# snap-stanford/pretrain-gnns

Hardware: NVIDIA H100
Metric: graphs/sec 5-layer GIN-300 fwd+bwd on ZINC-shaped batches (higher is better)
Workload: dtype tf32x3

## Files before the change

### include/pgnn_b200.h

```cpp
#ifndef PGNN_B200_H
#define PGNN_B200_H

#include <stdint.h>

#ifdef __cplusplus
extern "C" {
#endif

#define PGNN_API __attribute__((visibility("default")))

#define PGNN_OK 0
#define PGNN_EINVAL (-1)
#define PGNN_ECUDA (-2)
#define PGNN_EWORKSPACE (-3)
#define PGNN_EUNSUPPORTED (-4)

#define PGNN_DEVERR_NODE_ID 1u
#define PGNN_DEVERR_ATOM_CODE 2u
#define PGNN_DEVERR_BOND_CODE 4u
#define PGNN_DEVERR_LABEL 8u
#define PGNN_DEVERR_GATHER 16u

#define PGNN_AGG_SUM 0
#define PGNN_AGG_MEAN 1
#define PGNN_AGG_GCN 2

PGNN_API int pgnn_version(void);
PGNN_API const char* pgnn_error_string(int code);
PGNN_API int pgnn_last_cuda_error(void);
PGNN_API int pgnn_device_error_flags(int clear);
PGNN_API int pgnn_device_sm_count(int device);
PGNN_API int64_t pgnn_kernel_launch_count(void);
PGNN_API int pgnn_profile_enable(int on);
PGNN_API int64_t pgnn_profile_read(char* buf, int64_t buflen);


PGNN_API int64_t pgnn_bucket_workspace_bytes(int64_t num_keys, int64_t num_buckets);
PGNN_API int pgnn_bucket(const int64_t* keys, int64_t key_stride, int64_t num_keys, int64_t num_buckets,
                         const int64_t* vals, int64_t val_stride,
                         int32_t* rowptr, int32_t* order, int32_t* vals_out,
                         void* workspace, int64_t workspace_bytes, void* stream);

PGNN_API int64_t pgnn_graph_prep_workspace_bytes(int64_t num_nodes, int64_t num_edges);
PGNN_API int pgnn_graph_prep(const int64_t* edge_index, int64_t num_edges, int64_t num_nodes,
                             int32_t* rowptr_t, int32_t* nbr_t, int32_t* eid_t,
                             int32_t* rowptr_s, int32_t* nbr_s, int32_t* eid_s,
                             void* workspace, int64_t workspace_bytes, void* stream);

PGNN_API int pgnn_gcn_dinv(const int32_t* rowptr_t, int64_t num_nodes, float* dinv, void* stream);

PGNN_API int pgnn_chem_edge_summary(const int64_t* edge_attr , const int32_t* rowptr_t,
                                    const int32_t* nbr_t, const int32_t* eid_t, int64_t num_nodes,
                                    int mode, const float* dinv, float* S , void* stream);
PGNN_API int pgnn_bio_edge_summary(const float* edge_attr , const int32_t* rowptr_t,
                                   const int32_t* nbr_t, const int32_t* eid_t, int64_t num_nodes,
                                   int mode, const float* dinv, float* S , void* stream);

PGNN_API int pgnn_chem_embed_fwd(const int64_t* x , const float* tab1, int64_t rows1, const float* tab2, int64_t rows2,
                                 int64_t num_nodes, int64_t C, float* out, int64_t ldo, void* stream);
PGNN_API int pgnn_chem_embed_bwd(const int64_t* x, const float* g, int64_t ldg, int64_t num_nodes, int64_t C,
                                 float* gtab1, int64_t rows1, float* gtab2, int64_t rows2, void* stream);
PGNN_API int pgnn_bio_embed_fwd(const float* x , const float* tab , int64_t num_nodes,
                                int64_t C, float* out, int64_t ldo, void* stream);
PGNN_API int pgnn_bio_embed_bwd(const float* x, const float* g, int64_t ldg, int64_t num_nodes, int64_t C,
                                float* gtab , void* stream);

PGNN_API int pgnn_aggregate_fwd(const float* x, int64_t ldx, const float* in_scale, const float* in_shift,
                                int in_relu, int64_t num_nodes, int64_t C,
                                const int32_t* rowptr_t, const int32_t* nbr_t, int mode, const float* dinv,
                                const float* S, int64_t Q, const float* T , int64_t edge_off,
                                float* out, int64_t ldo, void* stream);
PGNN_API int pgnn_aggregate_bwd(const float* g, int64_t ldg, int64_t num_nodes, int64_t C,
                                const int32_t* rowptr_s, const int32_t* nbr_s, int mode, const float* dinv,
                                const int32_t* rowptr_t, float* gx, int64_t ldgx, void* stream);
PGNN_API int pgnn_edge_table_bwd(const float* S, int64_t Q, const float* g, int64_t ldg, int64_t g_off,
                                 int64_t num_nodes, int64_t C, float* gT, void* stream);

PGNN_API int pgnn_linear_fwd(const float* x, int64_t ldx, const float* w, const float* bias,
                             int64_t M, int64_t N, int64_t K, int relu, float* y, int64_t ldy,
                             int precision, void* stream);
PGNN_API int pgnn_linear_bwd_x(const float* gy, int64_t ldgy, const float* w, int64_t M, int64_t N, int64_t K,
                               const float* relu_src, int64_t ldr, float* gx, int64_t ldgx,
                               int precision, void* stream);
PGNN_API int pgnn_linear_bwd_w(const float* gy, int64_t ldgy, const float* x, int64_t ldx,
                               int64_t M, int64_t N, int64_t K, float* gw, float* gb,
                               int precision, void* stream);

PGNN_API int64_t pgnn_bn_workspace_bytes(int64_t M, int64_t C);
PGNN_API int pgnn_bn_fwd_train(const float* x, int64_t ldx, int64_t M, int64_t C, const float* gamma,
                               const float* beta, float* running_mean, float* running_var,
                               int64_t* num_batches_tracked, float momentum, float eps, int relu,
                               float* y, int64_t ldy, float* save_mean, float* save_invstd,
                               float* scale, float* shift, void* workspace, int64_t workspace_bytes,
                               void* stream);
PGNN_API int pgnn_bn_fwd_eval(const float* x, int64_t ldx, int64_t M, int64_t C, const float* gamma,
                              const float* beta, const float* running_mean, const float* running_var,
                              float eps, int relu, float* y, int64_t ldy, void* stream);
PGNN_API int pgnn_bn_bwd(const float* gy, int64_t ldgy, const float* x, int64_t ldx, int64_t M, int64_t C,
                         const float* gamma, const float* beta, const float* save_mean,
                         const float* save_invstd, int relu, float* gx, int64_t ldgx, float* ggamma,
                         float* gbeta, void* workspace, int64_t workspace_bytes, void* stream);
PGNN_API int pgnn_relu_fwd(const float* x, int64_t ldx, int64_t M, int64_t C, float* y, int64_t ldy, void* stream);
PGNN_API int pgnn_relu_bwd(const float* gy, int64_t ldgy, const float* y, int64_t ldy_, int64_t M, int64_t C,
                           float* gx, int64_t ldgx, void* stream);
PGNN_API int pgnn_dropout_fwd(const float* x, int64_t ldx, int64_t M, int64_t C, float p, int64_t seed, int64_t layer, float* y,
                              int64_t ldy, void* stream);
PGNN_API int pgnn_dropout_bwd(const float* gy, int64_t ldgy, int64_t M, int64_t C, float p, int64_t seed, int64_t layer, float* gx,
                              int64_t ldgx, void* stream);
PGNN_API int pgnn_l2norm_fwd(const float* x, int64_t ldx, int64_t M, int64_t C, float* y, int64_t ldy,
                             float* norm , void* stream);
PGNN_API int pgnn_l2norm_bwd(const float* gy, int64_t ldgy, const float* y, int64_t ldy_, const float* norm,
                             int64_t M, int64_t C, float* gx, int64_t ldgx, void* stream);

PGNN_API int pgnn_gat_fwd(const float* xl, int64_t num_nodes, int64_t H, int64_t D, const float* att ,
                          const float* T, int is_bio, const void* feat, const int32_t* rowptr_t,
                          const int32_t* nbr_t, const int32_t* eid_t, int64_t num_edges, const float* bias ,
                          float slope, float* alpha, float* pq, float* out , int64_t ldo, void* stream);
PGNN_API int64_t pgnn_gat_bwd_workspace_bytes(int64_t num_nodes, int64_t num_edges, int64_t H, int64_t D);
PGNN_API int pgnn_gat_bwd(const float* g , int64_t ldg, const float* xl, int64_t num_nodes, int64_t H,
                          int64_t D, const float* att, const float* T, int is_bio, const void* feat,
                          const int32_t* rowptr_t, const int32_t* nbr_t, const int32_t* eid_t,
                          const int32_t* rowptr_s, const int32_t* nbr_s, const int32_t* eid_s,
                          int64_t num_edges, float slope, const float* alpha, const float* pq,
                          float* gxl, float* gatt, float* gT, float* gbias,
                          void* workspace, int64_t workspace_bytes, void* stream);

PGNN_API int pgnn_segment_mean_fwd(const float* x, int64_t ldx, const int32_t* seg_ptr, const int32_t* seg_order,
                                   int64_t num_seg, int64_t C, float* out, int64_t ldo, void* stream);
PGNN_API int pgnn_segment_mean_bwd(const float* g, int64_t ldg, const int64_t* seg, const int32_t* seg_ptr,
                                   int64_t num_rows, int64_t C, float* gx, int64_t ldgx, void* stream);
PGNN_API int pgnn_row_gather_fwd(const float* x, int64_t ldx, int64_t num_rows, const int64_t* idx, const int64_t* idx2,
                                 int64_t num_idx, int64_t C, float* out, int64_t ldo, void* stream);
PGNN_API int pgnn_row_gather_bwd(const float* g, int64_t ldg, const int64_t* idx, const int64_t* idx2,
                                 int64_t num_idx, int64_t C, float* gx, int64_t ldgx, int64_t num_rows, void* stream);
PGNN_API int pgnn_softmax_ce_fwd(const float* logits, int64_t ld, int64_t M, int64_t V, const int64_t* labels,
                                 double* loss_mean, float* dlogits, int64_t lddl, void* stream);
PGNN_API int64_t pgnn_softmax_ce_rows_workspace_bytes(void);
PGNN_API int pgnn_softmax_ce_rows_fwd(const float* logits, int64_t ld, int64_t M, int64_t V, const float* label_rows, int64_t ld_label,
                                      int64_t Q, double* loss_mean, float* dlogits, int64_t lddl, void* workspace,
                                      int64_t workspace_bytes, void* stream);
PGNN_API int64_t pgnn_edge_pair_bce_workspace_bytes(void);
PGNN_API int pgnn_edge_pair_bce_fwd(const float* x, int64_t ldx, int64_t N, int64_t C, const int64_t* pos_u, const int64_t* pos_v,
                                    int64_t pos_stride, int64_t P, const int64_t* neg_u, const int64_t* neg_v, int64_t neg_stride,
                                    int64_t Q, double* loss, float* pos_scores, float* neg_scores, float* dscore, int64_t* pairs,
                                    void* workspace, int64_t workspace_bytes, void* stream);
PGNN_API int pgnn_edge_pair_bce_bwd(const float* x, int64_t ldx, int64_t N, int64_t C, const float* dscore, const double* gscale,
                                    const int32_t* rowptr_t, const int32_t* nbr_t, const int32_t* eid_t, const int32_t* rowptr_s,
                                    const int32_t* nbr_s, const int32_t* eid_s, float* gx, int64_t ldgx, void* stream);
PGNN_API int pgnn_infomax_summary_fwd(const float* x, int64_t ldx, const int32_t* seg_ptr, const int32_t* seg_order, int64_t G,
                                      int64_t C, float* S, int64_t lds, void* stream);
PGNN_API int64_t pgnn_infomax_bce_workspace_bytes(void);
PGNN_API int pgnn_infomax_bce_fwd(const float* x, int64_t ldx, int64_t N, int64_t C, const int64_t* batch, const float* H, int64_t G,
                                  double* loss, float* pos, float* neg, float* dscore, void* workspace, int64_t workspace_bytes,
                                  void* stream);
PGNN_API int64_t pgnn_infomax_bce_bwd_workspace_bytes(int64_t G, int64_t C);
PGNN_API int pgnn_infomax_bce_bwd(const float* x, int64_t ldx, int64_t N, int64_t C, const int64_t* batch, const int32_t* seg_ptr,
                                  const int32_t* seg_order, int64_t G, const float* S, const float* H, const float* W,
                                  const float* dscore, const double* gscale, float* gx, int64_t ldgx, float* gW, int precision,
                                  void* workspace, int64_t workspace_bytes, void* stream);
PGNN_API int pgnn_shifted_rowdot_fwd(const float* a, int64_t lda, const float* b, int64_t ldb, int64_t B, int64_t C,
                                     int64_t shift, float* out, void* stream);
PGNN_API int pgnn_shifted_rowdot_bwd(const float* g, const float* a, int64_t lda, const float* b, int64_t ldb,
                                     int64_t B, int64_t C, int64_t shift, int accumulate,
                                     float* ga, int64_t ldga, float* gb, int64_t ldgb, void* stream);
PGNN_API int64_t pgnn_bce_logits_workspace_bytes(void);
PGNN_API int pgnn_bce_logits_fwd(const float* logits, int64_t ld, int64_t M, int64_t N, const int64_t* target, int64_t ldt,
                                 int target_kind, double const_target, double* loss_mean, float* dlogits, int64_t lddl,
                                 void* workspace, int64_t workspace_bytes, void* stream);

PGNN_API int64_t pgnn_chem_gin_num_params(int64_t L);
PGNN_API int pgnn_chem_gin_grad_offsets(int64_t L, int64_t D, int64_t* offsets);
PGNN_API int64_t pgnn_chem_gin_workspace_bytes(int64_t N, int64_t E, int64_t L, int64_t D);
PGNN_API int pgnn_chem_gin_debug_layout(int64_t N, int64_t E, int64_t L, int64_t D, int64_t* out4);
PGNN_API int64_t pgnn_chem_gin_debug_aggr_offset(int64_t N, int64_t E, int64_t L, int64_t D);
PGNN_API int pgnn_debug_tc_gemm(int a_kc, int b_kc, int bn, const float* A, int64_t lda, const float* B, int64_t ldb, float* C,
                                int64_t ldc, int64_t M, int64_t N, int64_t K, const float* bias, int relu, const float* mask,
                                int64_t ldm, float* colsum, double* stats, const float* S, int Q, float* gT, float* gT2,
                                int q_split, int64_t ldt, void* stream);
PGNN_API int pgnn_debug_tc_wgrad(const float* gy, int64_t ldgy, const float* x, int64_t ldx, int64_t M, int64_t N, int64_t K,
                                 float* gw, float* gb, float* partials, int64_t partial_floats, void* stream);
PGNN_API int pgnn_debug_tc_wgrad_plan(int64_t M, int64_t N, int64_t K, int64_t* out4);
PGNN_API int pgnn_debug_transpose_batch(int count, const float* const* in, float* const* out, const int32_t* rows,
                                        const int32_t* cols, void* stream);
PGNN_API int pgnn_debug_bn_apply_fold(const float* x, int64_t ldx, int64_t M, int64_t C, const double* sums, const float* gamma,
                                      const float* beta, float* running_mean, float* running_var, int64_t* num_batches_tracked,
                                      float momentum, float eps, float* save_mean, float* save_invstd, int relu, float* y, int64_t ldy,
                                      float drop_p, int64_t drop_seed, int64_t drop_layer, void* stream);
PGNN_API int pgnn_debug_bn_bwd_colsum(const float* gy, int64_t ldgy, const float* x, int64_t ldx, int64_t M, int64_t C,
                                      const float* gamma, const float* beta, const float* save_mean, const float* save_invstd, int relu,
                                      float* gx, int64_t ldgx, float* ggamma, float* gbeta, float* colsum, float drop_p,
                                      int64_t drop_seed, int64_t drop_layer, void* workspace, int64_t workspace_bytes, void* stream);
PGNN_API int pgnn_chem_gin_forward(const void* const* params, void* const* bn_running_mean, void* const* bn_running_var,
                                   void* const* bn_num_batches_tracked, const int64_t* x, const int64_t* edge_index,
                                   const int64_t* edge_attr, int64_t N, int64_t E, int64_t L, int64_t D, int training,
                                   float momentum, float eps, int precision, float* node_rep, int64_t ld_out,
                                   void* workspace, int64_t workspace_bytes, void* stream);
PGNN_API int pgnn_chem_gin_backward(const void* const* params, const float* g_node_rep, int64_t ldg, const int64_t* x,
                                    int64_t N, int64_t E, int64_t L, int64_t D, int precision, float* grads,
                                    void* workspace, int64_t workspace_bytes, void* stream);

#define PGNN_CONV_GCN 1
#define PGNN_CONV_SAGE 2
#define PGNN_CONV_GAT 3
PGNN_API int64_t pgnn_chem_conv_num_params(int conv_type, int64_t L);
PGNN_API int pgnn_chem_conv_grad_offsets(int conv_type, int64_t L, int64_t D, int64_t* offsets);
PGNN_API int64_t pgnn_chem_conv_workspace_bytes(int conv_type, int64_t N, int64_t E, int64_t L, int64_t D);
PGNN_API int pgnn_chem_conv_forward(int conv_type, const void* const* params, void* const* bn_running_mean,
                                    void* const* bn_running_var, void* const* bn_num_batches_tracked, const int64_t* x,
                                    const int64_t* edge_index, const int64_t* edge_attr, int64_t N, int64_t E, int64_t L,
                                    int64_t D, int training, float momentum, float eps, int precision, float* node_rep,
                                    int64_t ld_out, void* workspace, int64_t workspace_bytes, void* stream);
PGNN_API int pgnn_chem_conv_backward(int conv_type, const void* const* params, const float* g_node_rep, int64_t ldg,
                                     const int64_t* x, const int64_t* edge_attr, int64_t N, int64_t E, int64_t L, int64_t D,
                                     int precision, float* grads, void* workspace, int64_t workspace_bytes, void* stream);

PGNN_API int pgnn_chem_encoder_forward(int gnn_type, const void* const* params, void* const* bn_running_mean,
                                       void* const* bn_running_var, void* const* bn_num_batches_tracked, const int64_t* x,
                                       const int64_t* edge_index, const int64_t* edge_attr, int64_t N, int64_t E, int64_t L,
                                       int64_t D, int training, float momentum, float eps, float drop_p, int64_t drop_seed,
                                       int precision, float* node_rep, int64_t ld_out, void* workspace, int64_t workspace_bytes,
                                       void* stream);
PGNN_API int pgnn_chem_encoder_backward(int gnn_type, const void* const* params, const float* g_node_rep, int64_t ldg,
                                        const int64_t* x, const int64_t* edge_attr, int64_t N, int64_t E, int64_t L, int64_t D,
                                        float drop_p, int64_t drop_seed, int precision, float* grads, void* workspace,
                                        int64_t workspace_bytes, void* stream);

PGNN_API int64_t pgnn_bio_encoder_num_params(int gnn_type, int64_t L);
PGNN_API int pgnn_bio_encoder_grad_offsets(int gnn_type, int64_t L, int64_t D, int64_t* offsets);
PGNN_API int64_t pgnn_bio_encoder_workspace_bytes(int gnn_type, int64_t N, int64_t E, int64_t L, int64_t D);
PGNN_API int pgnn_bio_encoder_forward(int gnn_type, const void* const* params, void* const* bn_running_mean,
                                      void* const* bn_running_var, void* const* bn_num_batches_tracked, const float* x ,
                                      const int64_t* edge_index, const float* edge_attr , int64_t N, int64_t E, int64_t L,
                                      int64_t D, int training, float momentum, float eps, float drop_p, int64_t drop_seed,
                                      int precision, float* node_rep, int64_t ld_out, void* workspace, int64_t workspace_bytes,
                                      void* stream);
PGNN_API int pgnn_bio_encoder_backward(int gnn_type, const void* const* params, const float* g_node_rep, int64_t ldg,
                                       const float* x, const float* edge_attr, int64_t N, int64_t E, int64_t L, int64_t D,
                                       float drop_p, int64_t drop_seed, int precision, float* grads, void* workspace,
                                       int64_t workspace_bytes, void* stream);

PGNN_API int pgnn_collate_chem(const int64_t* node_ptr, const int64_t* edge_ptr, const uint8_t* store_x,
                               const int32_t* store_edge_index, int64_t store_num_edges, const uint8_t* store_edge_attr,
                               const int64_t* graph_ids, int64_t B, int64_t* node_off, int64_t* edge_off, int64_t* x,
                               int64_t* edge_index, int64_t* edge_attr, int64_t* batch, void* stream);

PGNN_API int64_t pgnn_mask_atoms_count(const int64_t* node_off_host, int64_t B, double mask_rate);
PGNN_API int pgnn_mask_atoms(int64_t* x, const int64_t* node_off, int64_t B, double mask_rate, int64_t mask_token, int64_t seed,
                             int64_t* mask_off, int64_t* masked_atom_indices, int64_t* mask_node_label, void* stream);
PGNN_API int pgnn_collate_lists(const int64_t* list_ptr, const int32_t* values, const int64_t* graph_ids, int64_t B,
                                const int64_t* add_per_graph, int64_t* list_off, int64_t* out, int64_t* seg, int64_t* sizes,
                                void* stream);
PGNN_API int pgnn_collate_bio(const int64_t* node_ptr, const int64_t* edge_ptr, const int32_t* store_edge_index,
                              int64_t store_num_edges, const uint16_t* store_edge_bits, const int64_t* graph_ids, int64_t B,
                              int64_t* node_off, int64_t* edge_off, float* x, int64_t* edge_index, float* edge_attr,
                              int64_t* batch, void* stream);

PGNN_API int64_t pgnn_mask_edges_chem_workspace_bytes(int64_t N, int64_t B);
PGNN_API int pgnn_mask_edges_chem(const int64_t* edge_index, int64_t* edge_attr, const int64_t* edge_off, int64_t B, int64_t N,
                                  int64_t E, const int64_t* masked_atom_indices, int64_t M, int64_t num_edge_type,
                                  void* workspace, int64_t workspace_bytes, int64_t* conn_off, int64_t* connected_edge_indices,
                                  int64_t* mask_edge_label, void* stream);
PGNN_API int64_t pgnn_mask_edges_bio_count(const int64_t* edge_off_host, int64_t B, double mask_rate);
PGNN_API int pgnn_mask_edges_bio(float* edge_attr, const int64_t* edge_off, int64_t B, double mask_rate, int64_t seed,
                                 int64_t* mask_off, int64_t* masked_edge_idx, float* mask_edge_label, void* stream);
PGNN_API int64_t pgnn_negative_edges_capacity(const int64_t* edge_off_host, int64_t B);
PGNN_API int64_t pgnn_negative_edges_workspace_bytes(int64_t B, int64_t E, int64_t capacity);
PGNN_API int pgnn_negative_edges(const int64_t* edge_index, int64_t E, const int64_t* node_off, const int64_t* edge_off, int64_t B,
                                 int64_t seed, int64_t capacity, void* workspace, int64_t workspace_bytes, int64_t* negative_edge_index,
                                 int64_t* negative_edge_off, void* stream);

PGNN_API int64_t pgnn_extract_pairs_workspace_bytes(int64_t B, int64_t full_nodes);
PGNN_API int pgnn_extract_pairs(const int64_t* node_ptr, const int64_t* edge_ptr, const int32_t* store_edge_index,
                                int64_t store_num_edges, const uint8_t* pair_first, const int64_t* graph_ids, int64_t B,
                                int64_t full_nodes, const int32_t* roots, int64_t seed, int k, int l1, int l2, int whole_graph,
                                void* workspace, int64_t workspace_bytes, int64_t* offsets, void* stream);
PGNN_API int pgnn_extract_fill_chem(const int64_t* node_ptr, const int64_t* edge_ptr, const uint8_t* store_x,
                                    const int32_t* store_edge_index, int64_t store_num_edges, const uint8_t* store_edge_attr,
                                    const uint8_t* pair_first, const int64_t* graph_ids, int64_t B, int64_t full_nodes,
                                    const void* workspace, const int64_t* offsets, int64_t* x_substruct,
                                    int64_t* edge_index_substruct, int64_t* edge_attr_substruct, int64_t* center_substruct_idx,
                                    int64_t* x_context, int64_t* edge_index_context, int64_t* edge_attr_context,
                                    int64_t* overlap_context_substruct_idx, int64_t* batch_overlapped_context,
                                    int64_t* overlapped_context_size, void* stream);
PGNN_API int pgnn_extract_fill_bio(const int64_t* node_ptr, const int64_t* edge_ptr, const int32_t* store_edge_index,
                                   int64_t store_num_edges, const uint16_t* store_edge_bits, const uint8_t* pair_first,
                                   const int64_t* graph_ids, int64_t B, int64_t full_nodes, const void* workspace,
                                   const int64_t* offsets, float* x_context, int64_t* edge_index_context,
                                   float* edge_attr_context, int64_t* overlap_context_substruct_idx,
                                   int64_t* batch_overlapped_context, int64_t* overlapped_context_size, void* stream);

typedef struct PgnnAdamChunk {
  float* param;
  const float* grad;
  float* exp_avg;
  float* exp_avg_sq;
  int64_t n;
} PgnnAdamChunk;
PGNN_API int pgnn_adam_step(const PgnnAdamChunk* chunks, int64_t num_chunks, double lr, double beta1, double beta2, double eps,
                            double weight_decay, double grad_scale, int64_t step, int legacy_eps, void* stream);

PGNN_API int64_t pgnn_allreduce_p2p_scratch_floats(int64_t n, int world);
PGNN_API int pgnn_allreduce_p2p(void* const* bufs, void* const* flags, int rank, int world, int64_t n, float scale,
                                float* scratch, int64_t scratch_floats, int64_t epoch, void* stream);
PGNN_API int pgnn_allreduce_fused(void* const* in, void* const* out, void* const* flags, float* mc_in, float* mc_out,
                                  unsigned int* counter, int rank, int world, int64_t n, float scale, int64_t epoch, void* stream);
PGNN_API int pgnn_allreduce_nvls(float* mc_buf, void* const* flags, int rank, int world, int64_t n, float scale,
                                 int64_t epoch, void* stream);

#ifdef __cplusplus
}
#endif
#endif
```

### pretrain-gnns_b200/csrc/dense_tc.cu

```cuda
#include <cstdlib>

#include "common.cuh"

namespace {

constexpr int BM = 128;
constexpr int BK = 32;
constexpr int NTHREADS = 256;

__device__ __forceinline__ uint32_t smem_u32(const void* p) { return (uint32_t)__cvta_generic_to_shared(p); }

__device__ __forceinline__ int sw128_off(int r, int k) { return (r >> 3) * 1024 + (r & 7) * 128 + ((((k >> 2) ^ (r & 7))) << 4) + (k & 3) * 4; }

__device__ __forceinline__ uint64_t gmma_desc_sw128(uint32_t saddr) {
  return (uint64_t)((saddr & 0x3FFFFu) >> 4) | ((uint64_t)1 << 16) | ((uint64_t)(1024 >> 4) << 32) | ((uint64_t)1 << 62);
}

__device__ __forceinline__ void wgmma_fence() { asm volatile("wgmma.fence.sync.aligned;" ::: "memory"); }
__device__ __forceinline__ void wgmma_commit() { asm volatile("wgmma.commit_group.sync.aligned;" ::: "memory"); }
template <int N>
__device__ __forceinline__ void wgmma_wait() { asm volatile("wgmma.wait_group.sync.aligned %0;" ::"n"(N) : "memory"); }

__device__ __forceinline__ void wgmma_tf32_m64n64k8_rs(float (&d)[32], const uint32_t (&a)[4], uint64_t db) {
  asm volatile(
      "{\n\t"
      ".reg .pred p;\n\t"
      "setp.ne.b32 p, 1, 0;\n\t"
      "wgmma.mma_async.sync.aligned.m64n64k8.f32.tf32.tf32 "
      "{%0, %1, %2, %3, %4, %5, %6, %7, %8, %9, %10, %11, %12, %13, %14, %15, "
      "%16, %17, %18, %19, %20, %21, %22, %23, %24, %25, %26, %27, %28, %29, %30, %31}, {%32, %33, %34, %35}, %36, p, 1, 1;\n\t"
      "}\n"
      : "+f"(d[0]), "+f"(d[1]), "+f"(d[2]), "+f"(d[3]), "+f"(d[4]), "+f"(d[5]), "+f"(d[6]), "+f"(d[7]), "+f"(d[8]), "+f"(d[9]),
        "+f"(d[10]), "+f"(d[11]), "+f"(d[12]), "+f"(d[13]), "+f"(d[14]), "+f"(d[15]), "+f"(d[16]), "+f"(d[17]), "+f"(d[18]),
        "+f"(d[19]), "+f"(d[20]), "+f"(d[21]), "+f"(d[22]), "+f"(d[23]), "+f"(d[24]), "+f"(d[25]), "+f"(d[26]), "+f"(d[27]),
        "+f"(d[28]), "+f"(d[29]), "+f"(d[30]), "+f"(d[31])
      : "r"(a[0]), "r"(a[1]), "r"(a[2]), "r"(a[3]), "l"(db)
      : "memory");
}
__device__ __forceinline__ void wgmma_tf32_m64n128k8_rs(float (&d)[64], const uint32_t (&a)[4], uint64_t db) {
  asm volatile(
      "{\n\t"
      ".reg .pred p;\n\t"
      "setp.ne.b32 p, 1, 0;\n\t"
      "wgmma.mma_async.sync.aligned.m64n128k8.f32.tf32.tf32 "
      "{%0, %1, %2, %3, %4, %5, %6, %7, %8, %9, %10, %11, %12, %13, %14, %15, "
      "%16, %17, %18, %19, %20, %21, %22, %23, %24, %25, %26, %27, %28, %29, %30, %31, "
      "%32, %33, %34, %35, %36, %37, %38, %39, %40, %41, %42, %43, %44, %45, %46, %47, "
      "%48, %49, %50, %51, %52, %53, %54, %55, %56, %57, %58, %59, %60, %61, %62, %63}, {%64, %65, %66, %67}, %68, p, 1, 1;\n\t"
      "}\n"
      : "+f"(d[0]), "+f"(d[1]), "+f"(d[2]), "+f"(d[3]), "+f"(d[4]), "+f"(d[5]), "+f"(d[6]), "+f"(d[7]), "+f"(d[8]), "+f"(d[9]),
        "+f"(d[10]), "+f"(d[11]), "+f"(d[12]), "+f"(d[13]), "+f"(d[14]), "+f"(d[15]), "+f"(d[16]), "+f"(d[17]), "+f"(d[18]),
        "+f"(d[19]), "+f"(d[20]), "+f"(d[21]), "+f"(d[22]), "+f"(d[23]), "+f"(d[24]), "+f"(d[25]), "+f"(d[26]), "+f"(d[27]),
        "+f"(d[28]), "+f"(d[29]), "+f"(d[30]), "+f"(d[31]), "+f"(d[32]), "+f"(d[33]), "+f"(d[34]), "+f"(d[35]), "+f"(d[36]),
        "+f"(d[37]), "+f"(d[38]), "+f"(d[39]), "+f"(d[40]), "+f"(d[41]), "+f"(d[42]), "+f"(d[43]), "+f"(d[44]), "+f"(d[45]),
        "+f"(d[46]), "+f"(d[47]), "+f"(d[48]), "+f"(d[49]), "+f"(d[50]), "+f"(d[51]), "+f"(d[52]), "+f"(d[53]), "+f"(d[54]),
        "+f"(d[55]), "+f"(d[56]), "+f"(d[57]), "+f"(d[58]), "+f"(d[59]), "+f"(d[60]), "+f"(d[61]), "+f"(d[62]), "+f"(d[63])
      : "r"(a[0]), "r"(a[1]), "r"(a[2]), "r"(a[3]), "l"(db)
      : "memory");
}
template <int BN>
__device__ __forceinline__ void wgmma_tf32_rs(float (&d)[BN / 2], const uint32_t (&a)[4], uint64_t db) {
  if constexpr (BN == 128) wgmma_tf32_m64n128k8_rs(d, a, db);
  else wgmma_tf32_m64n64k8_rs(d, a, db);
}
template <int R>
__device__ __forceinline__ void fence_acc(float (&d)[R]) {
#pragma unroll
  for (int i = 0; i < R; ++i) asm volatile("" : "+f"(d[i])::"memory");
}

__device__ __forceinline__ int kperm(int k) { return (k & 16) | ((k & 3) << 2) | ((k >> 2) & 3); }

__device__ __forceinline__ int araw_off(int m, int k) { return k * BM + (m ^ ((((k >> 2) & 3) << 3) ^ ((k & 1) << 4))); }

__device__ __forceinline__ int akc_off(int m, int k) { return m * BK + ((((k >> 2) ^ ((m & 1) << 2))) << 2) + (k & 3); }

__device__ __forceinline__ void cp_async16(float* dst, const float* src, int bytes) {
  asm volatile("cp.async.cg.shared.global [%0], [%1], 16, %2;" ::"r"(smem_u32(dst)), "l"(src), "r"(bytes) : "memory");
}
__device__ __forceinline__ void cp_async_commit() { asm volatile("cp.async.commit_group;" ::: "memory"); }
__device__ __forceinline__ void cp_async_wait_all() { asm volatile("cp.async.wait_group 0;" ::: "memory"); }

__device__ __forceinline__ float tf32_trunc(float x) { return __uint_as_float(__float_as_uint(x) & 0xFFFFE000u); }

__device__ __forceinline__ void split_tf32(float x, float& hi, float& lo) {
  hi = tf32_trunc(__fadd_rn(x, 0.f));
  lo = x - hi;
}

__device__ __forceinline__ float sum_chains(float acc, float accx) { return isinf(acc) ? acc : acc + accx; }

__device__ __forceinline__ float4 ldg4_tail(const float* p, int n) {
  float4 x = make_float4(0.f, 0.f, 0.f, 0.f);
  if (n > 3) x = __ldg(reinterpret_cast<const float4*>(p));
  else if (n > 0) {
    x.x = __ldg(p);
    if (n > 1) x.y = __ldg(p + 1);
    if (n > 2) x.z = __ldg(p + 2);
  }
  return x;
}

__device__ __forceinline__ float f4_at(const float4& v, int i) { return i == 0 ? v.x : i == 1 ? v.y : i == 2 ? v.z : v.w; }

template <bool KC, int R>
struct Loader {
  static constexpr int NV = R * BK / 4 / NTHREADS;
  static_assert(NV >= 1 && R % 16 == 0, "tile rows");
  const float* base;
  int64_t ld, step;
  int r0, rows;
  float4 v[NV];

  __device__ __forceinline__ static void piece(int f, int& rr, int& kk) {
    if (KC) {
      rr = f >> 3;
      kk = (f & 7) * 4;
    } else {
      const int lane = f & 31, w = f >> 5, G = R / 16;
      rr = ((w % G) * 4 + (lane & 3)) * 4;
      kk = (w / G) * 8 + (lane >> 2);
    }
  }
  __device__ __forceinline__ void init(const float* __restrict__ src, int64_t ld_, int r0_, int rows_, int k0) {
    ld = ld_;
    r0 = r0_;
    rows = rows_;
    step = KC ? (int64_t)BK : (int64_t)BK * ld_;
    base = KC ? src + k0 : src + (int64_t)k0 * ld_;
  }
  __device__ __forceinline__ void load(int kb, int krem) {
    const float* blk = base + kb * step;
#pragma unroll
    for (int i = 0; i < NV; ++i) {
      int rr, kk;
      piece(threadIdx.x + i * NTHREADS, rr, kk);
      const int gr = r0 + rr;
      float4 x = make_float4(0.f, 0.f, 0.f, 0.f);
      if (KC) {
        if (gr < rows) x = ldg4_tail(blk + (int64_t)gr * ld + kk, krem - kk);
      } else if (kk < krem && gr < rows) {
        x = ldg4_tail(blk + (int64_t)kk * ld + gr, rows - gr);
      }
      v[i] = x;
    }
  }
  __device__ __forceinline__ void store(uint8_t* hi, uint8_t* lo) const {
#pragma unroll
    for (int i = 0; i < NV; ++i) {
      int rr, kk;
      piece(threadIdx.x + i * NTHREADS, rr, kk);
      if (!KC) asm volatile("" : "+r"(rr), "+r"(kk));
#pragma unroll
      for (int q = 0; q < 4; ++q) {
        float h, l;
        split_tf32(f4_at(v[i], q), h, l);
        const int o = KC ? sw128_off(rr, kperm(kk + q)) : sw128_off(rr + q, kperm(kk));
        *reinterpret_cast<float*>(hi + o) = h;
        *reinterpret_cast<float*>(lo + o) = l;
      }
    }
  }
};

template <bool KC>
__device__ __forceinline__ void a_copy(float* dst, const float* __restrict__ A, int64_t lda, int m0, int M, int k0, int krem) {
#pragma unroll
  for (int i = 0; i < Loader<KC, BM>::NV; ++i) {
    int rr, kk;
    Loader<KC, BM>::piece(threadIdx.x + i * NTHREADS, rr, kk);
    const int gr = m0 + rr;
    int n = 0;
    if (KC) n = gr < M ? min(max(krem - kk, 0), 4) : 0;
    else n = kk < krem ? min(max(M - gr, 0), 4) : 0;
    const float* src = n > 0 ? (KC ? A + (int64_t)gr * lda + k0 + kk : A + (int64_t)(k0 + kk) * lda + gr) : A;
    cp_async16(dst + (KC ? akc_off(rr, kk) : araw_off(rr, kk)), src, 4 * n);
  }
  cp_async_commit();
}

constexpr int NSTAGE = 3;

template <int BN>
struct TileCfg {
  static constexpr int B_BYTES = BN * BK * 4;
  static constexpr int STAGE = 2 * B_BYTES;
  static constexpr int A_RAW = BM * BK * 4;
  static constexpr int SLD = BN + 4;
  static constexpr int EPI = BM * SLD * 4 + BM * kMaxHookQ * 4;
  static constexpr int RING = NSTAGE * STAGE + 2 * A_RAW;
  static constexpr int SMEM = (RING > EPI ? RING : EPI) + 1024;
  static constexpr int FRAG_SETS = BN == 128 ? 4 : 2;
  static constexpr int MIN_BLOCKS = BN <= 64 ? 2 : 1;
};

template <int BN>
__device__ __forceinline__ void tile_epilogue(float* stage, const float* s_bias, bool s_bias_on, int m0, int n0, int M, int N,
                                              float* __restrict__ C, int64_t ldc, const TcEpilogue& ep) {
  constexpr int SLD = TileCfg<BN>::SLD;
  constexpr int C4 = BN / 4;
  constexpr int UNR = 4;
  const int rows_here = min(BM, M - m0);
  const int total = rows_here * C4;
  const bool vec_ok = ((ldc & 3) == 0) && ((reinterpret_cast<uintptr_t>(C) & 15) == 0);
  const bool mvec_ok = ep.mask_src && ((ep.ldm & 3) == 0) && ((reinterpret_cast<uintptr_t>(ep.mask_src) & 15) == 0);
  const bool want_hooks = ep.hooks.colsum || ep.hooks.stats || ep.hooks.S;
  for (int base = threadIdx.x; base < total; base += NTHREADS * UNR) {
    float4 o[UNR], mk[UNR];
    int gm[UNR], gn[UNR];
    bool live[UNR];
#pragma unroll
    for (int u = 0; u < UNR; ++u) {
      const int idx = base + u * NTHREADS;
      const int r = idx / C4, c4 = idx - r * C4;
      gm[u] = m0 + r;
      gn[u] = n0 + c4 * 4;
      live[u] = idx < total && gn[u] < N;
      mk[u] = make_float4(1.f, 1.f, 1.f, 1.f);
      if (live[u]) {
        o[u] = *reinterpret_cast<const float4*>(stage + r * SLD + c4 * 4);
        if (ep.mask_src) {
          const float* mp = ep.mask_src + (int64_t)gm[u] * ep.ldm + gn[u];
          if (mvec_ok && gn[u] + 3 < N) mk[u] = *reinterpret_cast<const float4*>(mp);
          else {
            mk[u].x = mp[0];
            mk[u].y = gn[u] + 1 < N ? mp[1] : 1.f;
            mk[u].z = gn[u] + 2 < N ? mp[2] : 1.f;
            mk[u].w = gn[u] + 3 < N ? mp[3] : 1.f;
          }
        }
      }
    }
#pragma unroll
    for (int u = 0; u < UNR; ++u) {
      if (!live[u]) continue;
      float ov[4] = {o[u].x, o[u].y, o[u].z, o[u].w};
      const float mv[4] = {mk[u].x, mk[u].y, mk[u].z, mk[u].w};
      const float4 b4 = s_bias_on ? *reinterpret_cast<const float4*>(s_bias + (gn[u] - n0)) : make_float4(0.f, 0.f, 0.f, 0.f);
      const float bv[4] = {b4.x, b4.y, b4.z, b4.w};
#pragma unroll
      for (int q = 0; q < 4; ++q) {
        if (s_bias_on) ov[q] += bv[q];
        if (ep.relu) ov[q] = relu_keep_nan(ov[q]);
        ov[q] = mv[q] > 0.f ? ov[q] : 0.f;
      }
      if (want_hooks)
        *reinterpret_cast<float4*>(stage + (gm[u] - m0) * SLD + (gn[u] - n0)) = make_float4(ov[0], ov[1], ov[2], ov[3]);
      float* dst = C + (int64_t)gm[u] * ldc + gn[u];
      if (gn[u] + 3 < N && vec_ok) {
        if (ep.atomic) atomicAdd(reinterpret_cast<float4*>(dst), make_float4(ov[0], ov[1], ov[2], ov[3]));
        else *reinterpret_cast<float4*>(dst) = make_float4(ov[0], ov[1], ov[2], ov[3]);
      } else {
#pragma unroll
        for (int q = 0; q < 4; ++q)
          if (gn[u] + q < N) {
            if (ep.atomic) atomicAdd(dst + q, ov[q]); else dst[q] = ov[q];
          }
      }
    }
  }
  if (want_hooks) {
    float* sS = stage + BM * SLD;
    if (ep.hooks.S)
      for (int i = threadIdx.x; i < rows_here * ep.hooks.Q; i += NTHREADS) sS[i] = ep.hooks.S[(int64_t)m0 * ep.hooks.Q + i];
    __syncthreads();
    const int c = threadIdx.x;
    if (c < BN && n0 + c < N) {
      const int Q = ep.hooks.Q;
      float s1 = 0.f;
      double d1 = 0.0, d2 = 0.0;
      float tq[kMaxHookQ];
#pragma unroll
      for (int q = 0; q < kMaxHookQ; ++q) tq[q] = 0.f;
      for (int r = 0; r < rows_here; ++r) {
        const float v = stage[r * SLD + c];
        s1 += v;
        if (ep.hooks.stats) { d1 += (double)v; d2 += (double)v * (double)v; }
        if (ep.hooks.S) {
#pragma unroll
          for (int q = 0; q < kMaxHookQ; ++q)
            if (q < Q) tq[q] = fmaf(sS[r * Q + q], v, tq[q]);
        }
      }
      if (ep.hooks.colsum) atomicAdd(&ep.hooks.colsum[n0 + c], s1);
      if (ep.hooks.stats) {
        atomicAdd(&ep.hooks.stats[n0 + c], d1);
        atomicAdd(&ep.hooks.stats[(int64_t)N + n0 + c], d2);
      }
      if (ep.hooks.S) {
#pragma unroll
        for (int q = 0; q < kMaxHookQ; ++q)
          if (q < Q)
            atomicAdd(q < ep.hooks.q_split ? &ep.hooks.gT[(int64_t)q * ep.hooks.ldt + n0 + c]
                                           : &ep.hooks.gT2[(int64_t)(q - ep.hooks.q_split) * ep.hooks.ldt + n0 + c], tq[q]);
      }
    }
  }
}

template <bool A_KC, bool B_KC, int BN>
__global__ void __launch_bounds__(NTHREADS, TileCfg<BN>::MIN_BLOCKS)
k_gemm_3xtf32(const float* __restrict__ A, int64_t lda, const float* __restrict__ B, int64_t ldb, float* __restrict__ C, int64_t ldc,
              int M, int N, int K, int k_per_split, TcEpilogue ep) {
  static_assert(BN == 64 || BN == 128, "one wgmma.m64nBNk8 per product; two accumulators of BN / 2 registers each");
  using Cfg = TileCfg<BN>;
  constexpr int NF = Cfg::FRAG_SETS;
  static_assert((BK / 8) % NF == 0, "k-step j uses fragment set j % NF in every block");
  extern __shared__ uint8_t smem_raw[];
  __shared__ __align__(16) float s_bias[BN];
  uint8_t* smem = smem_raw + ((1024 - (smem_u32(smem_raw) & 1023)) & 1023);
  auto b_hi = [&](int s) { return smem + s * Cfg::STAGE; };
  auto b_lo = [&](int s) { return b_hi(s) + Cfg::B_BYTES; };
  float* a_raw = reinterpret_cast<float*>(smem + NSTAGE * Cfg::STAGE);

  const int warp = threadIdx.x >> 5, lane = threadIdx.x & 31, wg = threadIdx.x >> 7;
  const int t = lane & 3;
  const int mrow = wg * 64 + (warp & 3) * 16 + (lane >> 2);
  const int m0 = blockIdx.y * BM, n0 = blockIdx.x * BN;
  const int kbeg = blockIdx.z * k_per_split;
  const int kend = min(K, kbeg + k_per_split);
  const int nkb = (kend - kbeg + BK - 1) / BK;
  const bool s_bias_on = ep.bias != nullptr && blockIdx.z == 0;

  pdl_prologue();
  for (int i = threadIdx.x; i < BN; i += NTHREADS) s_bias[i] = (s_bias_on && n0 + i < N) ? ep.bias[n0 + i] : 0.f;

  Loader<B_KC, BN> lb;
  lb.init(B, ldb, n0, N, kbeg);

  float acc[BN / 2], accx[BN / 2];
#pragma unroll
  for (int i = 0; i < BN / 2; ++i) acc[i] = accx[i] = 0.f;
  uint32_t fh[NF][4], fl[NF][4];

  if (nkb > 0) {
    a_copy<A_KC>(a_raw, A, lda, m0, M, kbeg, kend - kbeg);
    lb.load(0, kend - kbeg);
    lb.store(b_hi(0), b_lo(0));
    asm volatile("fence.proxy.async.shared::cta;" ::: "memory");
    cp_async_wait_all();
  }
  int s = 0;
#pragma unroll 1
  for (int kb = 0; kb < nkb; ++kb) {
    __syncthreads();
    const bool more = kb + 1 < nkb;
    if (more) {
      a_copy<A_KC>(a_raw + ((kb + 1) & 1) * (BM * BK), A, lda, m0, M, kbeg + (kb + 1) * BK, kend - kbeg - (kb + 1) * BK);
      lb.load(kb + 1, kend - kbeg - (kb + 1) * BK);
    }
    const float* ar = a_raw + (kb & 1) * (BM * BK);
    float4 av[2];
    const uint64_t dh = gmma_desc_sw128(smem_u32(b_hi(s))), dl = gmma_desc_sw128(smem_u32(b_lo(s)));
#pragma unroll
    for (int j = 0; j < BK / 8; ++j) {
      const int f = j % NF;
      wgmma_wait<NF - 1>();
      if (A_KC && (j & 1) == 0) {
#pragma unroll
        for (int r = 0; r < 2; ++r) av[r] = *reinterpret_cast<const float4*>(ar + akc_off(mrow + 8 * r, 16 * (j >> 1) + 4 * t));
      }
      float x[4];
#pragma unroll
      for (int q = 0; q < 4; ++q) {
        const int slot = 2 * (j & 1) + (q >> 1);
        if (A_KC) x[q] = f4_at(av[q & 1], slot);
        else x[q] = ar[araw_off(mrow + 8 * (q & 1), 16 * (j >> 1) + 4 * t + slot)];
      }
#pragma unroll
      for (int q = 0; q < 4; ++q) {
        float h, l;
        split_tf32(x[q], h, l);
        fh[f][q] = __float_as_uint(h);
        fl[f][q] = __float_as_uint(l);
      }
      wgmma_fence();
      wgmma_tf32_rs<BN>(accx, fl[f], dh + 2 * j);
      wgmma_tf32_rs<BN>(accx, fh[f], dl + 2 * j);
      wgmma_tf32_rs<BN>(acc, fh[f], dh + 2 * j);
      wgmma_commit();
    }
    s = s + 1 == NSTAGE ? 0 : s + 1;
    if (more) {
      lb.store(b_hi(s), b_lo(s));
      asm volatile("fence.proxy.async.shared::cta;" ::: "memory");
      cp_async_wait_all();
    }
  }
  wgmma_wait<0>();
  fence_acc(acc);
  fence_acc(accx);
  __syncthreads();

  float* stage = reinterpret_cast<float*>(smem);
#pragma unroll
  for (int i = 0; i < BN / 8; ++i) {
    const int col = i * 8 + t * 2;
    *reinterpret_cast<float2*>(stage + mrow * Cfg::SLD + col) =
        make_float2(sum_chains(acc[4 * i], accx[4 * i]), sum_chains(acc[4 * i + 1], accx[4 * i + 1]));
    *reinterpret_cast<float2*>(stage + (mrow + 8) * Cfg::SLD + col) =
        make_float2(sum_chains(acc[4 * i + 2], accx[4 * i + 2]), sum_chains(acc[4 * i + 3], accx[4 * i + 3]));
  }
  __syncthreads();
  tile_epilogue<BN>(stage, s_bias, s_bias_on, m0, n0, M, N, C + (int64_t)blockIdx.z * ep.split_stride, ldc, ep);
}

__global__ void __launch_bounds__(256)
k_colsum_tc(const float* __restrict__ gy, int64_t ld, int M, int N, int rows_per_block, float* __restrict__ gb) {
  pdl_prologue();
  __shared__ float red[8][33];
  const int lane = threadIdx.x & 31, w = threadIdx.x >> 5;
  const int n = blockIdx.x * 32 + lane;
  const int r0 = blockIdx.y * rows_per_block, r1 = min(M, r0 + rows_per_block);
  float a = 0.f;
  if (n < N) {
#pragma unroll 4
    for (int r = r0 + w; r < r1; r += 8) a += gy[(int64_t)r * ld + n];
  }
  red[w][lane] = a;
  __syncthreads();
  if (w == 0 && n < N) {
    float t = 0.f;
#pragma unroll
    for (int k = 0; k < 8; ++k) t += red[k][lane];
    atomicAdd(&gb[n], t);
  }
}

template <bool A_KC, bool B_KC, int BN>
int launch(const float* A, int64_t lda, const float* B, int64_t ldb, float* C, int64_t ldc, int M, int N, int K, int splits,
           int k_per_split, const TcEpilogue& ep, cudaStream_t st) {
  constexpr int smem = TileCfg<BN>::SMEM;
  static std::atomic<uint64_t> configured{0};
  int dev = 0;
  PGNN_CUDA(cudaGetDevice(&dev));
  const uint64_t bit = dev < 64 ? (uint64_t)1 << dev : 0;
  if (!(configured.load(std::memory_order_relaxed) & bit)) {
    PGNN_CUDA(cudaFuncSetAttribute(k_gemm_3xtf32<A_KC, B_KC, BN>, cudaFuncAttributeMaxDynamicSharedMemorySize, smem));
    configured.fetch_or(bit, std::memory_order_relaxed);
  }
  dim3 grid((unsigned)ceil_div(N, BN), (unsigned)ceil_div(M, BM), (unsigned)splits);
  PGNN_CUDA(pgnn_launch(k_gemm_3xtf32<A_KC, B_KC, BN>, dim3(grid), dim3(NTHREADS), smem, st, A, lda, B, ldb, C, ldc, M, N, K, k_per_split, ep));
  PGNN_LAUNCH_CHECK();
  return PGNN_OK;
}

inline int pick_bn(int M, int N, int splits) {
  const int64_t mt = ceil_div(M, BM) * (splits > 0 ? splits : 1);
  auto cost = [&](int bn, int per_sm) { return ceil_div(mt * ceil_div(N, bn), (int64_t)kNumSMs * per_sm) * bn * per_sm; };
  return cost(64, TileCfg<64>::MIN_BLOCKS) < cost(128, TileCfg<128>::MIN_BLOCKS) ? 64 : 128;
}

template <bool A_KC, bool B_KC>
int dispatch(int bn, const float* A, int64_t lda, const float* B, int64_t ldb, float* C, int64_t ldc, int M, int N, int K, int splits,
             int k_per_split, const TcEpilogue& ep, cudaStream_t st) {
  if (ep.hooks.S && (ep.hooks.Q < 1 || ep.hooks.Q > kMaxHookQ)) return PGNN_EINVAL;
  if (bn == 64) return launch<A_KC, B_KC, 64>(A, lda, B, ldb, C, ldc, M, N, K, splits, k_per_split, ep, st);
  return launch<A_KC, B_KC, 128>(A, lda, B, ldb, C, ldc, M, N, K, splits, k_per_split, ep, st);
}

}

extern "C" int pgnn_debug_tc_gemm(int a_kc, int b_kc, int bn, const float* A, int64_t lda, const float* B, int64_t ldb, float* C,
                                  int64_t ldc, int64_t M, int64_t N, int64_t K, const float* bias, int relu, const float* mask,
                                  int64_t ldm, float* colsum, double* stats, const float* S, int Q, float* gT, float* gT2,
                                  int q_split, int64_t ldt, void* stream) {
  PGNN_CHECK_ARG(bn == 64 || bn == 128);
  PGNN_CHECK_ARG(M > 0 && N > 0 && K > 0 && M < (1ll << 31) && N < (1ll << 31) && K < (1ll << 31));
  PGNN_CHECK_ARG(A && B && C && ldc >= N && lda >= (a_kc ? K : M) && ldb >= (b_kc ? K : N));
  PGNN_CHECK_ARG(!mask || ldm >= N);
  if (S) {
    PGNN_CHECK_ARG(Q >= 1 && Q <= kMaxHookQ && q_split >= 0 && q_split <= Q && ldt >= N);
    PGNN_CHECK_ARG((q_split == 0 || gT) && (q_split == Q || gT2));
  }
  if (lda % 4 || ldb % 4 || !aligned16(A) || !aligned16(B)) return PGNN_EUNSUPPORTED;
  TcEpilogue ep{bias, relu, mask, ldm, 0, PgnnGemmHooks{}};
  ep.hooks.colsum = colsum;
  ep.hooks.stats = stats;
  ep.hooks.S = S;
  ep.hooks.Q = S ? Q : 0;
  ep.hooks.gT = gT;
  ep.hooks.gT2 = gT2;
  ep.hooks.q_split = q_split;
  ep.hooks.ldt = ldt;
  cudaStream_t st = as_stream(stream);
  const int m = (int)M, n = (int)N, k = (int)K;
  if (a_kc && b_kc) return dispatch<true, true>(bn, A, lda, B, ldb, C, ldc, m, n, k, 1, k, ep, st);
  if (a_kc && !b_kc) return dispatch<true, false>(bn, A, lda, B, ldb, C, ldc, m, n, k, 1, k, ep, st);
  if (!a_kc && b_kc) return dispatch<false, true>(bn, A, lda, B, ldb, C, ldc, m, n, k, 1, k, ep, st);
  return dispatch<false, false>(bn, A, lda, B, ldb, C, ldc, m, n, k, 1, k, ep, st);
}

int pgnn_tc_linear_fwd(const float* x, int64_t ldx, const float* w, const float* bias, int64_t M, int64_t N, int64_t K, int relu,
                       float* y, int64_t ldy, cudaStream_t st, const PgnnGemmHooks* hooks) {
  if (K % 4 || ldx % 4 || !aligned16(x) || !aligned16(w) || !aligned16(y) || M < 1) return PGNN_EUNSUPPORTED;
  TcEpilogue ep{bias, relu, nullptr, 0, 0, hooks ? *hooks : PgnnGemmHooks{}};
  return dispatch<true, true>(pick_bn((int)M, (int)N, 1), x, ldx, w, K, y, ldy, (int)M, (int)N, (int)K, 1, (int)K, ep, st);
}

int pgnn_tc_linear_bwd_x(const float* gy, int64_t ldgy, const float* w, int64_t M, int64_t N, int64_t K, const float* relu_src,
                         int64_t ldr, float* gx, int64_t ldgx, cudaStream_t st, const PgnnGemmHooks* hooks) {
  if (K % 4 || ldgy % 4 || !aligned16(gy) || !aligned16(w) || !aligned16(gx) || M < 1) return PGNN_EUNSUPPORTED;
  TcEpilogue ep{nullptr, 0, relu_src, ldr, 0, hooks ? *hooks : PgnnGemmHooks{}};
  return dispatch<true, false>(pick_bn((int)M, (int)K, 1), gy, ldgy, w, K, gx, ldgx, (int)M, (int)K, (int)N, 1, (int)N, ep, st);
}

int pgnn_tc_linear_bwd_x_wt(const float* gy, int64_t ldgy, const float* wT, int64_t M, int64_t N, int64_t K, const float* relu_src,
                            int64_t ldr, float* gx, int64_t ldgx, cudaStream_t st, const PgnnGemmHooks* hooks) {
  if (N % 4 || ldgy % 4 || !aligned16(gy) || !aligned16(wT) || !aligned16(gx) || M < 1) return PGNN_EUNSUPPORTED;
  TcEpilogue ep{nullptr, 0, relu_src, ldr, 0, hooks ? *hooks : PgnnGemmHooks{}};
  return dispatch<true, true>(pick_bn((int)M, (int)K, 1), gy, ldgy, wT, N, gx, ldgx, (int)M, (int)K, (int)N, 1, (int)N, ep, st);
}

namespace {
struct TransposeJob { const float* in; float* out; int rows, cols; };
constexpr int kMaxTransposeJobs = 32;
struct TransposeBatch { TransposeJob job[kMaxTransposeJobs]; };
__global__ void __launch_bounds__(256) k_transpose_batch(TransposeBatch b) {
  pdl_prologue();
  __shared__ float tile[32][33];
  const TransposeJob j = b.job[blockIdx.z];
  const int c0 = blockIdx.x * 32, r0 = blockIdx.y * 32;
  if (c0 >= j.cols || r0 >= j.rows) return;
  const int tx = threadIdx.x & 31, ty = threadIdx.x >> 5;
  for (int i = ty; i < 32; i += 8)
    if (r0 + i < j.rows && c0 + tx < j.cols) tile[i][tx] = j.in[(int64_t)(r0 + i) * j.cols + c0 + tx];
  __syncthreads();
  for (int i = ty; i < 32; i += 8)
    if (c0 + i < j.cols && r0 + tx < j.rows) j.out[(int64_t)(c0 + i) * j.rows + r0 + tx] = tile[tx][i];
}
}

int pgnn_internal_transpose_batch(int count, const float* const* in, float* const* out, const int* rows, const int* cols,
                                  cudaStream_t st) {
  if (count <= 0) return PGNN_OK;
  if (count > kMaxTransposeJobs) return PGNN_EUNSUPPORTED;
  TransposeBatch b;
  int mr = 0, mc = 0;
  for (int i = 0; i < count; ++i) {
    b.job[i] = TransposeJob{in[i], out[i], rows[i], cols[i]};
    mr = rows[i] > mr ? rows[i] : mr;
    mc = cols[i] > mc ? cols[i] : mc;
  }
  dim3 grid((unsigned)ceil_div(mc, 32), (unsigned)ceil_div(mr, 32), (unsigned)count);
  PGNN_CUDA(pgnn_launch(k_transpose_batch, dim3(grid), dim3(256), 0, st, b));
  PGNN_LAUNCH_CHECK();
  return PGNN_OK;
}

namespace {
__global__ void __launch_bounds__(256) k_splitk_reduce(const float* __restrict__ part, int splits, int64_t n4, float* __restrict__ out) {
  pdl_prologue();
  for (int64_t i = blockIdx.x * (int64_t)blockDim.x + threadIdx.x; i < n4; i += (int64_t)gridDim.x * blockDim.x) {
    const float4* p = reinterpret_cast<const float4*>(part) + i;
    float4 a = p[0];
    int s = 1;
    for (; s + 3 < splits; s += 4) {
      const float4 b0 = p[(int64_t)s * n4], b1 = p[(int64_t)(s + 1) * n4], b2 = p[(int64_t)(s + 2) * n4], b3 = p[(int64_t)(s + 3) * n4];
      a.x += b0.x; a.y += b0.y; a.z += b0.z; a.w += b0.w;
      a.x += b1.x; a.y += b1.y; a.z += b1.z; a.w += b1.w;
      a.x += b2.x; a.y += b2.y; a.z += b2.z; a.w += b2.w;
      a.x += b3.x; a.y += b3.y; a.z += b3.z; a.w += b3.w;
    }
    for (; s < splits; ++s) {
      const float4 b = p[(int64_t)s * n4];
      a.x += b.x; a.y += b.y; a.z += b.z; a.w += b.w;
    }
    reinterpret_cast<float4*>(out)[i] = a;
  }
}

struct WgradPlan { int bn, tiles, splits, per; };
WgradPlan wgrad_plan(int64_t M, int64_t N, int64_t K) {
  WgradPlan p;
  p.bn = 128;
  if ((int)ceil_div(K, 128) * 128 > K + K * 15 / 100) p.bn = 64;
  p.tiles = (int)(ceil_div(N, BM) * ceil_div(K, p.bn));
  int splits = kNumSMs * TileCfg<128>::MIN_BLOCKS / p.tiles;
  if (p.bn == 64) splits = kNumSMs * TileCfg<64>::MIN_BLOCKS / p.tiles;
  if (splits < (int)ceil_div(M, 1024)) splits = (int)ceil_div(M, 1024);
  const int max_splits = (int)ceil_div(M, 2 * BK);
  if (splits > max_splits) splits = max_splits;
  if (splits < 1) splits = 1;
  p.per = (int)align_up(ceil_div(M, splits), BK);
  p.splits = (int)ceil_div(M, p.per);
  return p;
}
}

int64_t pgnn_tc_wgrad_workspace_floats(int64_t M, int64_t N, int64_t K) {
  if (M < 1) M = 1;
  const WgradPlan p = wgrad_plan(M, N, K);
  return (int64_t)p.splits * N * K;
}

int pgnn_tc_linear_bwd_w_ws(const float* gy, int64_t ldgy, const float* x, int64_t ldx, int64_t M, int64_t N, int64_t K, float* gw,
                            float* gb, float* partials, int64_t partial_floats, cudaStream_t st) {
  if (K % 4 || ldgy % 4 || ldx % 4 || !aligned16(gy) || !aligned16(x) || !aligned16(gw) || M < 1) return PGNN_EUNSUPPORTED;
  const WgradPlan plan = wgrad_plan(M, N, K);
  const int bn = plan.bn, splits = plan.splits, per = plan.per;
  int rc;
  if (splits > 1 && partials && aligned16(partials) && partial_floats >= (int64_t)splits * N * K && ((N * K) % 4 == 0)) {
    TcEpilogue ep{nullptr, 0, nullptr, 0, 0, PgnnGemmHooks{}};
    ep.split_stride = N * K;
    rc = dispatch<false, false>(bn, gy, ldgy, x, ldx, partials, K, (int)N, (int)K, (int)M, splits, per, ep, st);
    if (rc != PGNN_OK) return rc;
    const int64_t n4 = N * K / 4;
    int blocks = (int)ceil_div(n4, 256);
    if (blocks > kNumSMs * 4) blocks = kNumSMs * 4;
    PGNN_CUDA(pgnn_launch(k_splitk_reduce, dim3(blocks), dim3(256), 0, st, partials, splits, n4, gw));
    PGNN_LAUNCH_CHECK();
  } else {
    if (splits > 1) PGNN_CUDA(cudaMemsetAsync(gw, 0, sizeof(float) * N * K, st));
    TcEpilogue ep{nullptr, 0, nullptr, 0, splits > 1, PgnnGemmHooks{}};
    rc = dispatch<false, false>(bn, gy, ldgy, x, ldx, gw, K, (int)N, (int)K, (int)M, splits, per, ep, st);
    if (rc != PGNN_OK) return rc;
  }
  if (gb) {
    PGNN_CUDA(cudaMemsetAsync(gb, 0, sizeof(float) * N, st));
    const int rows_per = M >= 16384 ? 256 : 64;
    dim3 g2((unsigned)ceil_div(N, 32), (unsigned)ceil_div(M, rows_per));
    PGNN_CUDA(pgnn_launch(k_colsum_tc, dim3(g2), dim3(256), 0, st, gy, ldgy, (int)M, (int)N, rows_per, gb));
    PGNN_LAUNCH_CHECK();
  }
  return PGNN_OK;
}

int pgnn_tc_linear_bwd_w(const float* gy, int64_t ldgy, const float* x, int64_t ldx, int64_t M, int64_t N, int64_t K, float* gw,
                         float* gb, cudaStream_t st) {
  return pgnn_tc_linear_bwd_w_ws(gy, ldgy, x, ldx, M, N, K, gw, gb, nullptr, 0, st);
}

extern "C" {

int pgnn_debug_tc_wgrad(const float* gy, int64_t ldgy, const float* x, int64_t ldx, int64_t M, int64_t N, int64_t K, float* gw,
                        float* gb, float* partials, int64_t partial_floats, void* stream) {
  PGNN_CHECK_ARG(M > 0 && N > 0 && K > 0 && M < (1ll << 31) && N < (1ll << 31) && K < (1ll << 31));
  PGNN_CHECK_ARG(gy && x && gw && ldgy >= N && ldx >= K && partial_floats >= 0);
  return pgnn_tc_linear_bwd_w_ws(gy, ldgy, x, ldx, M, N, K, gw, gb, partials, partial_floats, as_stream(stream));
}

int pgnn_debug_tc_wgrad_plan(int64_t M, int64_t N, int64_t K, int64_t* out4) {
  PGNN_CHECK_ARG(M > 0 && N > 0 && K > 0 && M < (1ll << 31) && N < (1ll << 31) && K < (1ll << 31) && out4);
  const WgradPlan p = wgrad_plan(M, N, K);
  out4[0] = p.bn;
  out4[1] = p.tiles;
  out4[2] = p.splits;
  out4[3] = p.per;
  return PGNN_OK;
}

int pgnn_debug_transpose_batch(int count, const float* const* in, float* const* out, const int32_t* rows, const int32_t* cols,
                               void* stream) {
  PGNN_CHECK_ARG(count >= 0);
  if (count == 0) return PGNN_OK;
  PGNN_CHECK_ARG(in && out && rows && cols);
  if (count > kMaxTransposeJobs) return PGNN_EUNSUPPORTED;
  for (int i = 0; i < count; ++i) PGNN_CHECK_ARG(in[i] && out[i] && rows[i] > 0 && cols[i] > 0);
  return pgnn_internal_transpose_batch(count, in, out, rows, cols, as_stream(stream));
}

}
```

### pretrain-gnns_b200/csrc/encoder.cu

```cuda
#include "common.cuh"

#include <cstdlib>
#include <map>
#include <mutex>
#include <vector>

int pgnn_internal_edge_table_bwd2(const float* S, int Q, const float* g, int64_t ldg, int64_t g_off, int64_t n, int C, float* gT,
                                  int64_t ldt, float* gT2, int q_split, cudaStream_t st);
int pgnn_internal_aggregate_fwd(const float* x, int64_t ldx, const float* in_scale, const float* in_shift, int in_relu,
                                int64_t num_nodes, int64_t C, const int32_t* rowptr_t, const int32_t* nbr_t, int mode, const float* dinv,
                                const float* S, int64_t Q, const float* T, const float* T2, int q_split, int64_t edge_off, float* out,
                                int64_t ldo, cudaStream_t st, const PgnnBnFold* fold, const PgnnDropout* drop);

int pgnn_internal_chem_onehot(const int64_t* x, int64_t n, int rows1, int rows2, float* onehot, int64_t ld, cudaStream_t st);

int pgnn_tc_linear_fwd(const float*, int64_t, const float*, const float*, int64_t, int64_t, int64_t, int, float*, int64_t,
                       cudaStream_t, const PgnnGemmHooks*);
int pgnn_tc_linear_bwd_x(const float*, int64_t, const float*, int64_t, int64_t, int64_t, const float*, int64_t, float*, int64_t,
                         cudaStream_t, const PgnnGemmHooks*);
int pgnn_tc_linear_bwd_w(const float*, int64_t, const float*, int64_t, int64_t, int64_t, int64_t, float*, float*, cudaStream_t);
int pgnn_tc_linear_bwd_w_ws(const float* gy, int64_t ldgy, const float* x, int64_t ldx, int64_t M, int64_t N, int64_t K, float* gw,
                            float* gb, float* partials, int64_t partial_floats, cudaStream_t st);
int64_t pgnn_tc_wgrad_workspace_floats(int64_t M, int64_t N, int64_t K);
int pgnn_tc_linear_bwd_x_wt(const float* gy, int64_t ldgy, const float* wT, int64_t M, int64_t N, int64_t K, const float* relu_src,
                            int64_t ldr, float* gx, int64_t ldgx, cudaStream_t st, const PgnnGemmHooks* hooks);
int pgnn_internal_transpose_batch(int count, const float* const* in, float* const* out, const int* rows, const int* cols,
                                  cudaStream_t st);
int pgnn_internal_bn_apply_fold(const float* x, int64_t ldx, int64_t M, int64_t C, const PgnnBnFold& fold, int relu, float* y,
                                int64_t ldy, cudaStream_t st, const PgnnDropout* drop);
int pgnn_internal_bn_fwd_train(const float* x, int64_t ldx, int64_t M, int64_t C, const float* gamma, const float* beta,
                               float* running_mean, float* running_var, int64_t* num_batches_tracked, float momentum, float eps,
                               int relu, float* y, int64_t ldy, float* save_mean, float* save_invstd, float* scale, float* shift,
                               void* workspace, int64_t workspace_bytes, void* stream, const PgnnDropout* drop);
int pgnn_internal_bn_bwd(const float* gy, int64_t ldgy, const float* x, int64_t ldx, int64_t M, int64_t C, const float* gamma,
                         const float* beta, const float* save_mean, const float* save_invstd, int relu, float* gx, int64_t ldgx,
                         float* ggamma, float* gbeta, float* colsum, void* workspace, int64_t workspace_bytes, cudaStream_t st,
                         const PgnnDropout* drop);

namespace {

constexpr int kGin = 0;
constexpr int kAtomRows = 120, kChiralRows = 3;
constexpr int kOneHotLd = 124;
constexpr int kHeads = 2;
constexpr float kSlope = 0.2f;

enum { P_XEMB1 = 0, P_XEMB2 = 1, P_LAYER0 = 2 };
enum { L_W1 = 0, L_B1, L_W2, L_B2, L_ET1, L_ET2, L_GAMMA, L_BETA, L_COUNT };
enum { G_W = 0, G_B, G_ET1, G_ET2, G_GAMMA, G_BETA, G_COUNT };
enum { A_W = 0, A_B, A_ATT, A_BIAS, A_ET1, A_ET2, A_GAMMA, A_BETA, A_COUNT };

inline int layer_params(int type) { return type == kGin ? L_COUNT : type == PGNN_CONV_GAT ? A_COUNT : G_COUNT; }
inline int agg_mode(int type) { return type == kGin ? PGNN_AGG_SUM : type == PGNN_CONV_GCN ? PGNN_AGG_GCN : PGNN_AGG_MEAN; }
bool valid_conv(int t) { return t == PGNN_CONV_GCN || t == PGNN_CONV_SAGE || t == PGNN_CONV_GAT; }

struct Drops {
  float p = 0.f;
  int64_t seed = 0;
  PgnnDropout at(int64_t l) const {
    PgnnDropout d;
    pgnn_make_dropout(p, seed, l, &d);
    return d;
  }
};

#define TRY(call)                     \
  do {                                \
    int rc__ = (call);                \
    if (rc__ != PGNN_OK) return rc__; \
  } while (0)

int64_t grad_layout(int type, int64_t L, int64_t D, int64_t* offsets) {
  if (!offsets) return 2 + (int64_t)layer_params(type) * L;
  const int64_t HD = type == PGNN_CONV_GAT ? kHeads * D : D;
  int64_t o = 0, i = 0;
  auto next = [&](int64_t size) { offsets[i++] = o; o += size; };
  next(kAtomRows * D);
  next(kChiralRows * D);
  for (int64_t l = 0; l < L; ++l) {
    if (type == kGin) {
      next(2 * D * D);
      next(2 * D);
      next(2 * D * D);
      next(D);
    } else {
      next(HD * D);
      next(HD);
      if (type == PGNN_CONV_GAT) {
        next(kHeads * 2 * D);
        next(D);
      }
    }
    next(6 * HD);
    next(3 * HD);
    next(D);
    next(D);
  }
  offsets[i] = o;
  return i;
}

struct Carve {
  char* base;
  bool pad_empty;
  int64_t off = 0;
  Carve(void* b, bool pad) : base(reinterpret_cast<char*>(b)), pad_empty(pad) {}
  template <typename T>
  T* take(int64_t count) {
    T* p = reinterpret_cast<T*>(base + off);
    off += align_up((pad_empty && count < 1 ? 1 : count) * (int64_t)sizeof(T), 256);
    return p;
  }
};

struct Front {
  int32_t *rowptr_t, *rowptr_s, *nbr_t, *eid_t, *nbr_s, *eid_s;
  float *S, *dinv, *h0;
  float* onehot;
};

void carve_front(Carve& c, Front& f, int type, int64_t N, int64_t E, int64_t D, int64_t Q = 9, int64_t onehot_ld = kOneHotLd) {
  const int64_t e1 = E > 0 ? E : 1;
  f.rowptr_t = c.take<int32_t>(N + 1);
  f.rowptr_s = c.take<int32_t>(N + 1);
  f.nbr_t = c.take<int32_t>(e1);
  f.eid_t = c.take<int32_t>(e1);
  f.nbr_s = c.take<int32_t>(e1);
  f.eid_s = c.take<int32_t>(e1);
  f.S = c.take<float>(N * Q);
  f.dinv = type == kGin ? nullptr : c.take<float>(N);
  f.h0 = c.take<float>(N * D);
  f.onehot = onehot_ld ? c.take<float>(N * onehot_ld) : nullptr;
}

int64_t split_k_floats(int64_t N, int64_t width, int64_t D) {
  const int64_t a = pgnn_tc_wgrad_workspace_floats(N, width, D);
  const int64_t e = pgnn_tc_wgrad_workspace_floats(N, kAtomRows + kChiralRows, D);
  return e > a ? e : a;
}

struct GinWs : Front {
  float *scale, *shift, *mean, *invstd;
  double* bn_acc;
  float *aggr, *z1, *z2;
  float *gh, *gz2, *gz1, *gaggr;
  float* wT;
  float* wpart;
  int64_t wpart_floats;
  void* scratch;
  int64_t scratch_bytes, total;
};

GinWs carve_gin(void* base, int64_t N, int64_t E, int64_t L, int64_t D) {
  Carve c(base, false);
  GinWs w;
  carve_front(c, w, kGin, N, E, D);
  w.bn_acc = c.take<double>(L * 2 * D);
  w.scale = c.take<float>(L * D);
  w.shift = c.take<float>(L * D);
  w.mean = c.take<float>(L * D);
  w.invstd = c.take<float>(L * D);
  w.aggr = c.take<float>(L * N * D);
  w.z1 = c.take<float>(L * N * 2 * D);
  w.z2 = c.take<float>(L * N * D);
  w.gh = c.take<float>(N * D);
  w.gz2 = c.take<float>(2 * N * D);
  w.gz1 = c.take<float>(2 * N * 2 * D);
  w.gaggr = c.take<float>(N * D);
  w.wT = c.take<float>(L * 4 * D * D);
  w.wpart_floats = split_k_floats(N, 2 * D, D);
  w.wpart = c.take<float>(w.wpart_floats);
  int64_t sb = pgnn_graph_prep_workspace_bytes(N, E);
  const int64_t bb = pgnn_bn_workspace_bytes(N > 0 ? N : 1, D);
  if (bb > sb) sb = bb;
  w.scratch_bytes = sb;
  w.scratch = c.take<char>(sb);
  w.total = c.off;
  return w;
}

struct ConvWs : Front {
  float *xl, *z, *hout;
  float *nrm, *alpha, *pq, *T;
  float *mean, *invstd;
  float *gz, *ga, *gxl, *gh;
  float* wpart;
  int64_t wpart_floats;
  void* scratch;
  int64_t scratch_bytes, total;
};

ConvWs carve_conv(void* base, int type, int64_t N, int64_t E, int64_t L, int64_t D) {
  Carve c(base, true);
  ConvWs w;
  const int64_t HD = type == PGNN_CONV_GAT ? kHeads * D : D;
  carve_front(c, w, type, N, E, D);
  w.xl = c.take<float>(L * N * HD);
  w.z = c.take<float>(L * N * D);
  w.hout = c.take<float>(L * N * D);
  w.nrm = c.take<float>(type == PGNN_CONV_SAGE ? L * N : 0);
  w.alpha = c.take<float>(type == PGNN_CONV_GAT ? L * (E + N) * kHeads : 0);
  w.pq = c.take<float>(type == PGNN_CONV_GAT ? L * N * kHeads * 2 : 0);
  w.T = c.take<float>(type == PGNN_CONV_GAT ? L * 9 * HD : 0);
  w.mean = c.take<float>(L * D);
  w.invstd = c.take<float>(L * D);
  w.gz = c.take<float>(N * D);
  w.ga = c.take<float>(N * D);
  w.gxl = c.take<float>(2 * N * HD);
  w.gh = c.take<float>(N * D);
  w.wpart_floats = split_k_floats(N, HD, D);
  w.wpart = c.take<float>(w.wpart_floats);
  int64_t sb = pgnn_graph_prep_workspace_bytes(N, E);
  const int64_t bb = pgnn_bn_workspace_bytes(N > 0 ? N : 1, D);
  if (bb > sb) sb = bb;
  if (type == PGNN_CONV_GAT) {
    const int64_t gb = pgnn_gat_bwd_workspace_bytes(N, E, kHeads, D);
    if (gb > sb) sb = gb;
  }
  w.scratch_bytes = sb;
  w.scratch = c.take<char>(sb);
  w.total = c.off;
  return w;
}

struct SideCtx {
  cudaStream_t side = nullptr;
  cudaEvent_t ready[2][2] = {}, done[2][2] = {}, join = nullptr;
  bool ok = false;
};
SideCtx* side_ctx(cudaStream_t main_stream) {
  static std::mutex mu;
  static std::map<std::pair<int, cudaStream_t>, SideCtx*> all;
  static int enabled = -1;
  std::lock_guard<std::mutex> g(mu);
  if (enabled < 0) {
    const char* e = getenv("PGNN_WGRAD_STREAM");
    enabled = (e && e[0] == '0') ? 0 : 1;
  }
  if (!enabled || g_pgnn_profile_on.load(std::memory_order_relaxed) != 0) return nullptr;
  int dev = 0;
  if (cudaGetDevice(&dev) != cudaSuccess) return nullptr;
  auto key = std::make_pair(dev, main_stream);
  auto it = all.find(key);
  if (it != all.end()) return it->second->ok ? it->second : nullptr;
  SideCtx* c = new SideCtx();
  all[key] = c;
  bool ok = cudaStreamCreateWithFlags(&c->side, cudaStreamNonBlocking) == cudaSuccess;
  for (int k = 0; k < 2 && ok; ++k)
    for (int i = 0; i < 2 && ok; ++i)
      ok = cudaEventCreateWithFlags(&c->ready[k][i], cudaEventDisableTiming) == cudaSuccess &&
           cudaEventCreateWithFlags(&c->done[k][i], cudaEventDisableTiming) == cudaSuccess;
  ok = ok && cudaEventCreateWithFlags(&c->join, cudaEventDisableTiming) == cudaSuccess;
  if (!ok) cudaGetLastError();
  c->ok = ok;
  return ok ? c : nullptr;
}

int join_side(const SideCtx* sc, cudaStream_t st) {
  PGNN_CUDA(cudaEventRecord(sc->join, sc->side));
  PGNN_CUDA(cudaStreamWaitEvent(st, sc->join, 0));
  return PGNN_OK;
}

int forward_prologue(int type, const Front& f, const void* const* params, const int64_t* x, const int64_t* edge_index,
                     const int64_t* edge_attr, int64_t N, int64_t E, int64_t D, int training, int precision, void* scratch,
                     int64_t scratch_bytes, void* stream) {
  TRY(pgnn_graph_prep(edge_index, E, N, f.rowptr_t, f.nbr_t, f.eid_t, f.rowptr_s, f.nbr_s, f.eid_s, scratch, scratch_bytes, stream));
  if (type == PGNN_CONV_GCN) TRY(pgnn_gcn_dinv(f.rowptr_t, N, f.dinv, stream));
  if (type != PGNN_CONV_GAT) TRY(pgnn_chem_edge_summary(edge_attr, f.rowptr_t, f.nbr_t, f.eid_t, N, agg_mode(type), f.dinv, f.S, stream));
  TRY(pgnn_chem_embed_fwd(x, (const float*)params[P_XEMB1], kAtomRows, (const float*)params[P_XEMB2], kChiralRows, N, D, f.h0, D, stream));
  if (training && precision == 1) TRY(pgnn_internal_chem_onehot(x, N, kAtomRows, kChiralRows, f.onehot, kOneHotLd, as_stream(stream)));
  return PGNN_OK;
}

int embed_backward(const SideCtx* sc, const Front& f, const float* gh, const int64_t* x, int64_t N, int64_t D, int precision,
                   float* grads, const int64_t* off, float* wpart, int64_t wpart_floats, cudaStream_t st) {
  if (sc) TRY(join_side(sc, st));
  int rc = PGNN_EUNSUPPORTED;
  if (precision == 1)
    rc = pgnn_tc_linear_bwd_w_ws(f.onehot, kOneHotLd, gh, D, N, kAtomRows + kChiralRows, D, grads + off[P_XEMB1], nullptr, wpart,
                                 wpart_floats, st);
  if (rc == PGNN_EUNSUPPORTED)
    rc = pgnn_chem_embed_bwd(x, gh, D, N, D, grads + off[P_XEMB1], kAtomRows, grads + off[P_XEMB2], kChiralRows, st);
  return rc;
}

int gin_forward(const void* const* params, void* const* bn_running_mean, void* const* bn_running_var, void* const* bn_num_batches_tracked,
                const int64_t* x, const int64_t* edge_index, const int64_t* edge_attr, int64_t N, int64_t E, int64_t L, int64_t D,
                int training, float momentum, float eps, const Drops& drops, int precision, float* node_rep, int64_t ld_out,
                void* workspace, int64_t workspace_bytes, void* stream) {
  PGNN_CHECK_ARG(N >= 0 && E >= 0 && L >= 1 && D > 0 && D % 4 == 0 && params && bn_running_mean && bn_running_var && workspace);
  PGNN_CHECK_ARG(N == 0 || (x && node_rep));
  if (workspace_bytes < pgnn_chem_gin_workspace_bytes(N, E, L, D)) return PGNN_EWORKSPACE;
  if (N == 0) return PGNN_OK;
  GinWs w = carve_gin(workspace, N, E, L, D);
  TRY(forward_prologue(kGin, w, params, x, edge_index, edge_attr, N, E, D, training, precision, w.scratch, w.scratch_bytes, stream));
  const float* h = w.h0;
  const float *in_scale = nullptr, *in_shift = nullptr;
  PgnnBnFold fold;
  bool have_fold = false;
  double* const bn_acc = w.bn_acc;
  for (int64_t l = 0; l < L; ++l) {
    const void* const* p = params + P_LAYER0 + l * L_COUNT;
    float* aggr = w.aggr + l * N * D;
    float* z1 = w.z1 + l * N * 2 * D;
    float* z2 = w.z2 + l * N * D;
    const bool last = (l == L - 1);
    const PgnnDropout drop_in = drops.at(l > 0 ? l - 1 : 0), drop_out = drops.at(l);
    TRY(pgnn_internal_aggregate_fwd(h, D, in_scale, in_shift, in_scale != nullptr || have_fold, N, D, w.rowptr_t, w.nbr_t, PGNN_AGG_SUM,
                                    nullptr, w.S, 9, (const float*)p[L_ET1], (const float*)p[L_ET2], 6, 0, aggr, D, as_stream(stream),
                                    have_fold ? &fold : nullptr, l > 0 ? &drop_in : nullptr));
    TRY(pgnn_linear_fwd(aggr, D, (const float*)p[L_W1], (const float*)p[L_B1], N, 2 * D, D, 1, z1, 2 * D, precision, stream));
    have_fold = false;
    bool stats_fused = false;
    double* acc = bn_acc + l * 2 * D;
    if (training && precision == 1) {
      PGNN_CUDA(cudaMemsetAsync(acc, 0, sizeof(double) * 2 * D, as_stream(stream)));
      PgnnGemmHooks hk;
      hk.stats = acc;
      const int rc = pgnn_tc_linear_fwd(z1, 2 * D, (const float*)p[L_W2], (const float*)p[L_B2], N, D, 2 * D, 0, z2, D, as_stream(stream), &hk);
      if (rc == PGNN_OK) stats_fused = true;
      else if (rc != PGNN_EUNSUPPORTED) return rc;
    }
    if (!stats_fused)
      TRY(pgnn_linear_fwd(z1, 2 * D, (const float*)p[L_W2], (const float*)p[L_B2], N, D, 2 * D, 0, z2, D, precision, stream));
    if (training && stats_fused) {
      fold = PgnnBnFold{};
      fold.acc = acc; fold.gamma = (const float*)p[L_GAMMA]; fold.beta = (const float*)p[L_BETA];
      fold.running_mean = (float*)bn_running_mean[l]; fold.running_var = (float*)bn_running_var[l];
      fold.nbt = bn_num_batches_tracked ? (int64_t*)bn_num_batches_tracked[l] : nullptr;
      fold.save_mean = w.mean + l * D; fold.save_invstd = w.invstd + l * D;
      fold.momentum = momentum; fold.eps = eps; fold.set_rows((int)N);
      if (last) {
        TRY(pgnn_internal_bn_apply_fold(z2, D, N, D, fold, 0, node_rep, ld_out, as_stream(stream), &drop_out));
      } else {
        have_fold = true;
      }
      h = z2;
      in_scale = in_shift = nullptr;
    } else if (training) {
      TRY(pgnn_internal_bn_fwd_train(z2, D, N, D, (const float*)p[L_GAMMA], (const float*)p[L_BETA], (float*)bn_running_mean[l],
                                     (float*)bn_running_var[l], bn_num_batches_tracked ? (int64_t*)bn_num_batches_tracked[l] : nullptr,
                                     momentum, eps, 0, last ? node_rep : nullptr, ld_out, w.mean + l * D, w.invstd + l * D, w.scale + l * D,
                                     w.shift + l * D, w.scratch, w.scratch_bytes, stream, &drop_out));
      h = z2;
      in_scale = w.scale + l * D;
      in_shift = w.shift + l * D;
    } else {
      float* y = last ? node_rep : ((l & 1) ? w.gz2 : w.gaggr);
      TRY(pgnn_bn_fwd_eval(z2, D, N, D, (const float*)p[L_GAMMA], (const float*)p[L_BETA], (const float*)bn_running_mean[l],
                           (const float*)bn_running_var[l], eps, !last, y, last ? ld_out : D, stream));
      h = y;
      in_scale = in_shift = nullptr;
    }
  }
  return PGNN_OK;
}

int gin_backward(const void* const* params, const float* g_node_rep, int64_t ldg, const int64_t* x, int64_t N, int64_t E, int64_t L,
                 int64_t D, const Drops& drops, int precision, float* grads, void* workspace, int64_t workspace_bytes, void* stream) {
  PGNN_CHECK_ARG(N >= 0 && E >= 0 && L >= 1 && D > 0 && D % 4 == 0 && params && grads && workspace);
  if (workspace_bytes < pgnn_chem_gin_workspace_bytes(N, E, L, D)) return PGNN_EWORKSPACE;
  const int64_t count = grad_layout(kGin, L, D, nullptr);
  std::vector<int64_t> offsets(count + 1);
  const int64_t* off = offsets.data();
  grad_layout(kGin, L, D, offsets.data());
  cudaStream_t st = as_stream(stream);
  if (N == 0) {
    PGNN_CUDA(cudaMemsetAsync(grads, 0, sizeof(float) * off[count], st));
    return PGNN_OK;
  }
  PGNN_CHECK_ARG(g_node_rep && x);
  GinWs w = carve_gin(workspace, N, E, L, D);
  bool have_wT = false;
  if (precision == 1 && 2 * L <= 32) {
    const float* in[32];
    float* out[32];
    int rows[32], cols[32];
    for (int64_t l = 0; l < L; ++l) {
      const void* const* p = params + P_LAYER0 + l * L_COUNT;
      in[2 * l] = (const float*)p[L_W1];     out[2 * l] = w.wT + (2 * l) * 2 * D * D;     rows[2 * l] = (int)(2 * D); cols[2 * l] = (int)D;
      in[2 * l + 1] = (const float*)p[L_W2]; out[2 * l + 1] = w.wT + (2 * l + 1) * 2 * D * D; rows[2 * l + 1] = (int)D; cols[2 * l + 1] = (int)(2 * D);
    }
    const int rc = pgnn_internal_transpose_batch((int)(2 * L), in, out, rows, cols, st);
    if (rc == PGNN_OK) have_wT = true;
    else if (rc != PGNN_EUNSUPPORTED) return rc;
  }
  const float* gy = g_node_rep;
  int64_t ldgy = ldg;
  SideCtx* sc = precision == 1 ? side_ctx(st) : nullptr;
  cudaStream_t wst = sc ? sc->side : st;
  for (int64_t l = L - 1; l >= 0; --l) {
    const void* const* p = params + P_LAYER0 + l * L_COUNT;
    const int64_t* o = off + P_LAYER0 + l * L_COUNT;
    const float* aggr = w.aggr + l * N * D;
    const float* z1 = w.z1 + l * N * 2 * D;
    const float* z2 = w.z2 + l * N * D;
    const bool last = (l == L - 1);
    const int par = (int)(l & 1);
    float* gz2 = w.gz2 + (sc ? par * N * D : 0);
    float* gz1 = w.gz1 + (sc ? par * N * 2 * D : 0);
    if (sc) PGNN_CUDA(cudaStreamWaitEvent(st, sc->done[0][par], 0));
    const PgnnDropout drop = drops.at(l);
    TRY(pgnn_internal_bn_bwd(gy, ldgy, z2, D, N, D, (const float*)p[L_GAMMA], (const float*)p[L_BETA], w.mean + l * D,
                             w.invstd + l * D, !last, gz2, D, grads + o[L_GAMMA], grads + o[L_BETA], grads + o[L_B2],
                             w.scratch, w.scratch_bytes, st, &drop));
    bool fused = false;
    if (precision == 1) {
      if (sc) {
        PGNN_CUDA(cudaEventRecord(sc->ready[0][par], st));
        PGNN_CUDA(cudaStreamWaitEvent(wst, sc->ready[0][par], 0));
      }
      int rc = pgnn_tc_linear_bwd_w_ws(gz2, D, z1, 2 * D, N, D, 2 * D, grads + o[L_W2], nullptr, w.wpart, w.wpart_floats, wst);
      if (rc == PGNN_OK) {
        if (sc) {
          PGNN_CUDA(cudaEventRecord(sc->done[0][par], wst));
          PGNN_CUDA(cudaStreamWaitEvent(st, sc->done[1][par], 0));
        }
        PGNN_CUDA(cudaMemsetAsync(grads + o[L_B1], 0, sizeof(float) * 2 * D, st));
        PgnnGemmHooks h1;
        h1.colsum = grads + o[L_B1];
        rc = have_wT ? pgnn_tc_linear_bwd_x_wt(gz2, D, w.wT + (2 * l + 1) * 2 * D * D, N, D, 2 * D, z1, 2 * D, gz1, 2 * D, st, &h1)
                     : PGNN_EUNSUPPORTED;
        if (rc == PGNN_EUNSUPPORTED)
          rc = pgnn_tc_linear_bwd_x(gz2, D, (const float*)p[L_W2], N, D, 2 * D, z1, 2 * D, gz1, 2 * D, st, &h1);
        if (rc != PGNN_OK) return rc;
        if (sc) {
          PGNN_CUDA(cudaEventRecord(sc->ready[1][par], st));
          PGNN_CUDA(cudaStreamWaitEvent(wst, sc->ready[1][par], 0));
        }
        rc = pgnn_tc_linear_bwd_w_ws(gz1, 2 * D, aggr, D, N, 2 * D, D, grads + o[L_W1], nullptr, w.wpart, w.wpart_floats, wst);
        if (rc != PGNN_OK) return rc;
        if (sc) PGNN_CUDA(cudaEventRecord(sc->done[1][par], wst));
        PGNN_CUDA(cudaMemsetAsync(grads + o[L_ET1], 0, sizeof(float) * 9 * D, st));
        PgnnGemmHooks h2;
        h2.S = w.S; h2.Q = 9; h2.gT = grads + o[L_ET1]; h2.gT2 = grads + o[L_ET2]; h2.q_split = 6; h2.ldt = D;
        rc = have_wT ? pgnn_tc_linear_bwd_x_wt(gz1, 2 * D, w.wT + (2 * l) * 2 * D * D, N, 2 * D, D, nullptr, 0, w.gaggr, D, st, &h2)
                     : PGNN_EUNSUPPORTED;
        if (rc == PGNN_EUNSUPPORTED)
          rc = pgnn_tc_linear_bwd_x(gz1, 2 * D, (const float*)p[L_W1], N, 2 * D, D, nullptr, 0, w.gaggr, D, st, &h2);
        if (rc != PGNN_OK) return rc;
        fused = true;
      } else if (rc != PGNN_EUNSUPPORTED) {
        return rc;
      }
    }
    if (!fused) {
      if (sc) TRY(join_side(sc, st));
      TRY(pgnn_linear_bwd_w(gz2, D, z1, 2 * D, N, D, 2 * D, grads + o[L_W2], nullptr, precision, stream));
      TRY(pgnn_linear_bwd_x(gz2, D, (const float*)p[L_W2], N, D, 2 * D, z1, 2 * D, gz1, 2 * D, precision, stream));
      TRY(pgnn_linear_bwd_w(gz1, 2 * D, aggr, D, N, 2 * D, D, grads + o[L_W1], grads + o[L_B1], precision, stream));
      TRY(pgnn_linear_bwd_x(gz1, 2 * D, (const float*)p[L_W1], N, 2 * D, D, nullptr, 0, w.gaggr, D, precision, stream));
      PGNN_CUDA(cudaMemsetAsync(grads + o[L_ET1], 0, sizeof(float) * 9 * D, st));
      TRY(pgnn_internal_edge_table_bwd2(w.S, 9, w.gaggr, D, 0, N, (int)D, grads + o[L_ET1], D, grads + o[L_ET2], 6, st));
    }
    TRY(pgnn_aggregate_bwd(w.gaggr, D, N, D, w.rowptr_s, w.nbr_s, PGNN_AGG_SUM, nullptr, w.rowptr_t, w.gh, D, stream));
    gy = w.gh;
    ldgy = D;
  }
  return embed_backward(sc, w, w.gh, x, N, D, precision, grads, off, w.wpart, w.wpart_floats, st);
}

int conv_forward(int conv_type, const void* const* params, void* const* bn_running_mean, void* const* bn_running_var,
                 void* const* bn_num_batches_tracked, const int64_t* x, const int64_t* edge_index, const int64_t* edge_attr, int64_t N,
                 int64_t E, int64_t L, int64_t D, int training, float momentum, float eps, const Drops& drops, int precision,
                 float* node_rep, int64_t ld_out, void* workspace, int64_t workspace_bytes, void* stream) {
  PGNN_CHECK_ARG(valid_conv(conv_type) && N >= 0 && E >= 0 && L >= 1 && D > 0 && D % 4 == 0 && params && bn_running_mean && bn_running_var &&
                 workspace);
  PGNN_CHECK_ARG(N == 0 || (x && node_rep));
  PGNN_CHECK_ARG(E == 0 || (edge_index && edge_attr));
  if (workspace_bytes < pgnn_chem_conv_workspace_bytes(conv_type, N, E, L, D)) return PGNN_EWORKSPACE;
  if (N == 0) return PGNN_OK;
  cudaStream_t st = as_stream(stream);
  const bool gat = conv_type == PGNN_CONV_GAT;
  const int64_t HD = gat ? kHeads * D : D;
  const int PL = layer_params(conv_type);
  ConvWs w = carve_conv(workspace, conv_type, N, E, L, D);
  TRY(forward_prologue(conv_type, w, params, x, edge_index, edge_attr, N, E, D, training, precision, w.scratch, w.scratch_bytes, stream));
  const float* h = w.h0;
  for (int64_t l = 0; l < L; ++l) {
    const void* const* p = params + P_LAYER0 + l * PL;
    const bool last = l == L - 1;
    float* xl = w.xl + l * N * HD;
    float* z = w.z + l * N * D;
    float* hout = last ? node_rep : w.hout + l * N * D;
    const int64_t ldh = last ? ld_out : D;
    TRY(pgnn_linear_fwd(h, D, (const float*)p[gat ? A_W : G_W], (const float*)p[gat ? A_B : G_B], N, HD, D, 0, xl, HD, precision, stream));
    if (gat) {
      float* T = w.T + l * 9 * HD;
      PGNN_CUDA(cudaMemcpyAsync(T, p[A_ET1], sizeof(float) * 6 * HD, cudaMemcpyDeviceToDevice, st));
      PGNN_CUDA(cudaMemcpyAsync(T + 6 * HD, p[A_ET2], sizeof(float) * 3 * HD, cudaMemcpyDeviceToDevice, st));
      TRY(pgnn_gat_fwd(xl, N, kHeads, D, (const float*)p[A_ATT], T, 0, edge_attr, w.rowptr_t, w.nbr_t, w.eid_t, E, (const float*)p[A_BIAS], kSlope,
                       w.alpha + l * (E + N) * kHeads, w.pq + l * N * kHeads * 2, z, D, stream));
    } else if (conv_type == PGNN_CONV_GCN) {
      TRY(pgnn_internal_aggregate_fwd(xl, D, nullptr, nullptr, 0, N, D, w.rowptr_t, w.nbr_t, PGNN_AGG_GCN, w.dinv, w.S, 9, (const float*)p[G_ET1],
                                      (const float*)p[G_ET2], 6, 0, z, D, st, nullptr, nullptr));
    } else {
      TRY(pgnn_internal_aggregate_fwd(xl, D, nullptr, nullptr, 0, N, D, w.rowptr_t, w.nbr_t, PGNN_AGG_MEAN, nullptr, w.S, 9, (const float*)p[G_ET1],
                                      (const float*)p[G_ET2], 6, 0, w.gz, D, st, nullptr, nullptr));
      TRY(pgnn_l2norm_fwd(w.gz, D, N, D, z, D, w.nrm + l * N, stream));
    }
    const float* gamma = (const float*)p[gat ? A_GAMMA : G_GAMMA];
    const float* beta = (const float*)p[gat ? A_BETA : G_BETA];
    if (training) {
      const PgnnDropout drop = drops.at(l);
      TRY(pgnn_internal_bn_fwd_train(z, D, N, D, gamma, beta, (float*)bn_running_mean[l], (float*)bn_running_var[l],
                                     bn_num_batches_tracked ? (int64_t*)bn_num_batches_tracked[l] : nullptr, momentum, eps, !last, hout, ldh,
                                     w.mean + l * D, w.invstd + l * D, nullptr, nullptr, w.scratch, w.scratch_bytes, stream, &drop));
    } else {
      TRY(pgnn_bn_fwd_eval(z, D, N, D, gamma, beta, (const float*)bn_running_mean[l], (const float*)bn_running_var[l], eps, !last, hout, ldh, stream));
    }
    h = hout;
  }
  return PGNN_OK;
}

int conv_backward(int conv_type, const void* const* params, const float* g_node_rep, int64_t ldg, const int64_t* x,
                  const int64_t* edge_attr, int64_t N, int64_t E, int64_t L, int64_t D, const Drops& drops, int precision, float* grads,
                  void* workspace, int64_t workspace_bytes, void* stream) {
  PGNN_CHECK_ARG(valid_conv(conv_type) && N >= 0 && E >= 0 && L >= 1 && D > 0 && D % 4 == 0 && params && grads && workspace);
  if (workspace_bytes < pgnn_chem_conv_workspace_bytes(conv_type, N, E, L, D)) return PGNN_EWORKSPACE;
  const int64_t count = grad_layout(conv_type, L, D, nullptr);
  std::vector<int64_t> offsets(count + 1);
  const int64_t* off = offsets.data();
  grad_layout(conv_type, L, D, offsets.data());
  cudaStream_t st = as_stream(stream);
  const bool gat = conv_type == PGNN_CONV_GAT;
  const int64_t HD = gat ? kHeads * D : D;
  const int PL = layer_params(conv_type);
  if (N == 0) {
    PGNN_CUDA(cudaMemsetAsync(grads, 0, sizeof(float) * off[count], st));
    return PGNN_OK;
  }
  PGNN_CHECK_ARG(g_node_rep && x && (E == 0 || edge_attr));
  ConvWs w = carve_conv(workspace, conv_type, N, E, L, D);
  const float* gy = g_node_rep;
  int64_t ldgy = ldg;
  SideCtx* sc = precision == 1 ? side_ctx(st) : nullptr;
  cudaStream_t wst = sc ? sc->side : st;
  for (int64_t l = L - 1; l >= 0; --l) {
    const void* const* p = params + P_LAYER0 + l * PL;
    const int64_t* o = off + P_LAYER0 + l * PL;
    const bool last = l == L - 1;
    const int par = (int)(l & 1);
    const float* xl = w.xl + l * N * HD;
    const float* z = w.z + l * N * D;
    const float* hin = l == 0 ? w.h0 : w.hout + (l - 1) * N * D;
    float* gxl = w.gxl + (sc ? par * N * HD : 0);
    const float* gamma = (const float*)p[gat ? A_GAMMA : G_GAMMA];
    const float* beta = (const float*)p[gat ? A_BETA : G_BETA];
    const PgnnDropout drop = drops.at(l);
    TRY(pgnn_internal_bn_bwd(gy, ldgy, z, D, N, D, gamma, beta, w.mean + l * D, w.invstd + l * D, !last, w.gz, D,
                             grads + o[gat ? A_GAMMA : G_GAMMA], grads + o[gat ? A_BETA : G_BETA], nullptr, w.scratch, w.scratch_bytes, st,
                             &drop));
    if (sc) PGNN_CUDA(cudaStreamWaitEvent(st, sc->done[0][par], 0));
    if (gat) {
      TRY(pgnn_gat_bwd(w.gz, D, xl, N, kHeads, D, (const float*)p[A_ATT], w.T + l * 9 * HD, 0, edge_attr, w.rowptr_t, w.nbr_t, w.eid_t, w.rowptr_s,
                       w.nbr_s, w.eid_s, E, kSlope, w.alpha + l * (E + N) * kHeads, w.pq + l * N * kHeads * 2, gxl, grads + o[A_ATT],
                       grads + o[A_ET1], grads + o[A_BIAS], w.scratch, w.scratch_bytes, stream));
    } else {
      const float* ga = w.gz;
      if (conv_type == PGNN_CONV_SAGE) {
        TRY(pgnn_l2norm_bwd(w.gz, D, z, D, w.nrm + l * N, N, D, w.ga, D, stream));
        ga = w.ga;
      }
      PGNN_CUDA(cudaMemsetAsync(grads + o[G_ET1], 0, sizeof(float) * 9 * D, st));
      TRY(pgnn_internal_edge_table_bwd2(w.S, 9, ga, D, 0, N, (int)D, grads + o[G_ET1], D, grads + o[G_ET2], 6, st));
      TRY(pgnn_aggregate_bwd(ga, D, N, D, w.rowptr_s, w.nbr_s, agg_mode(conv_type), w.dinv, w.rowptr_t, gxl, D, stream));
    }
    if (sc) {
      PGNN_CUDA(cudaEventRecord(sc->ready[0][par], st));
      PGNN_CUDA(cudaStreamWaitEvent(wst, sc->ready[0][par], 0));
    }
    int rc = PGNN_EUNSUPPORTED;
    if (precision == 1)
      rc = pgnn_tc_linear_bwd_w_ws(gxl, HD, hin, D, N, HD, D, grads + o[gat ? A_W : G_W], grads + o[gat ? A_B : G_B], w.wpart, w.wpart_floats, wst);
    if (rc == PGNN_EUNSUPPORTED) {
      if (sc) TRY(join_side(sc, st));
      rc = pgnn_linear_bwd_w(gxl, HD, hin, D, N, HD, D, grads + o[gat ? A_W : G_W], grads + o[gat ? A_B : G_B], precision, stream);
    } else if (sc) {
      PGNN_CUDA(cudaEventRecord(sc->done[0][par], wst));
    }
    if (rc != PGNN_OK) return rc;
    TRY(pgnn_linear_bwd_x(gxl, HD, (const float*)p[gat ? A_W : G_W], N, HD, D, nullptr, 0, w.gh, D, precision, stream));
    gy = w.gh;
    ldgy = D;
  }
  return embed_backward(sc, w, w.gh, x, N, D, precision, grads, off, w.wpart, w.wpart_floats, st);
}


constexpr int kBioQ = 10;
constexpr int kBioEmbRows = 2;
constexpr int kMaxPack = 64;

enum BioParam {
  PB_EMB = 0, PB_LAYER0 = 1,
  BG_W1 = 0, BG_B1, BG_GAMMA, BG_BETA, BG_W2, BG_B2, BG_ENC_W, BG_ENC_B, BG_COUNT,
  BC_W = 0, BC_B, BC_ENC_W, BC_ENC_B, BC_COUNT,
  BA_W = 0, BA_B, BA_ATT, BA_BIAS, BA_ENC_W, BA_ENC_B, BA_COUNT
};

inline int bio_layer_params(int type) { return type == kGin ? BG_COUNT : type == PGNN_CONV_GAT ? BA_COUNT : BC_COUNT; }
inline int bio_enc_w(int type) { return type == kGin ? BG_ENC_W : type == PGNN_CONV_GAT ? BA_ENC_W : BC_ENC_W; }
inline int64_t bio_width(int type, int64_t D) { return type == PGNN_CONV_GAT ? kHeads * D : D; }
bool valid_type(int t) { return t == kGin || valid_conv(t); }

int64_t bio_grad_layout(int type, int64_t L, int64_t D, int64_t* offsets) {
  if (!offsets) return 1 + (int64_t)bio_layer_params(type) * L;
  const int64_t C = bio_width(type, D);
  int64_t o = 0, i = 0;
  auto next = [&](int64_t size) { offsets[i++] = o; o += size; };
  next(kBioEmbRows * D);
  for (int64_t l = 0; l < L; ++l) {
    if (type == kGin) {
      next(4 * D * D);
      next(2 * D);
      next(2 * D);
      next(2 * D);
      next(2 * D * D);
      next(D);
    } else {
      next(C * D);
      next(C);
      if (type == PGNN_CONV_GAT) {
        next(kHeads * 2 * D);
        next(D);
      }
    }
    next(9 * C);
    next(C);
  }
  offsets[i] = o;
  return i;
}

struct PackArgs {
  const float* w[kMaxPack];
  const float* b[kMaxPack];
};

__global__ void __launch_bounds__(256) k_bio_pack_tables(PackArgs a, int count, int C, float* __restrict__ T) {
  pdl_prologue();
  const int64_t per = (int64_t)kBioQ * C, total = per * count;
  for (int64_t idx = blockIdx.x * (int64_t)blockDim.x + threadIdx.x; idx < total; idx += (int64_t)gridDim.x * blockDim.x) {
    const int l = (int)(idx / per);
    const int r = (int)(idx - l * per);
    const int q = r / C, c = r - q * C;
    T[idx] = q < 9 ? a.w[l][c * 9 + q] : a.b[l][c];
  }
}

__global__ void __launch_bounds__(256) k_bio_unpack_table_grads(const float* __restrict__ gT, int64_t L, int C, float* __restrict__ out,
                                                                int64_t stride) {
  pdl_prologue();
  const int64_t per = (int64_t)kBioQ * C, total = per * L;
  for (int64_t idx = blockIdx.x * (int64_t)blockDim.x + threadIdx.x; idx < total; idx += (int64_t)gridDim.x * blockDim.x) {
    const int64_t l = idx / per;
    const int r = (int)(idx - l * per);
    const int q = r / C, c = r - q * C;
    out[l * stride + (q < 9 ? (int64_t)c * 9 + q : (int64_t)9 * C + c)] = gT[idx];
  }
}

__device__ __forceinline__ float bio_act1(float v, float z, bool bwd, int relu) {
  return relu ? (bwd ? (z > 0.f ? v : 0.f) : relu_keep_nan(v)) : v;
}

template <bool BWD, bool DROP, int VEC>
__global__ void __launch_bounds__(256) k_bio_act(const float* __restrict__ x, int64_t ldx, const float* __restrict__ z, int64_t ldz,
                                                 int64_t M, int64_t C, int relu, PgnnDropout d, float* __restrict__ y, int64_t ldy) {
  pdl_prologue();
  const int lane = threadIdx.x & 31;
  const int64_t warps = (int64_t)gridDim.x * (blockDim.x >> 5);
  for (int64_t r = blockIdx.x * (int64_t)(blockDim.x >> 5) + (threadIdx.x >> 5); r < M; r += warps) {
    for (int64_t c = (int64_t)lane * VEC; c < C; c += 32 * VEC) {
      if (VEC == 4) {
        float4 v = ld4(x + r * ldx + c);
        const float4 zz = BWD && relu ? ld4(z + r * ldz + c) : v;
        v.x = bio_act1(v.x, zz.x, BWD, relu);
        v.y = bio_act1(v.y, zz.y, BWD, relu);
        v.z = bio_act1(v.z, zz.z, BWD, relu);
        v.w = bio_act1(v.w, zz.w, BWD, relu);
        if (DROP) v = dropout4(v, d, r, C, c);
        st4(y + r * ldy + c, v);
      } else {
        float v = bio_act1(x[r * ldx + c], BWD && relu ? z[r * ldz + c] : 0.f, BWD, relu);
        if (DROP) v *= dropout_factor(d, r, C, c);
        y[r * ldy + c] = v;
      }
    }
  }
}

int bio_act(bool bwd, const float* x, int64_t ldx, const float* z, int64_t ldz, int64_t M, int64_t C, int relu, const PgnnDropout& d,
            float* y, int64_t ldy, cudaStream_t st) {
  const bool drop = d.p > 0.f;
  const bool v4 = C % 4 == 0 && ldx % 4 == 0 && ldy % 4 == 0 && aligned16(x) && aligned16(y) &&
                  (!(bwd && relu) || (ldz % 4 == 0 && aligned16(z)));
  auto k = v4 ? (bwd ? (drop ? k_bio_act<true, true, 4> : k_bio_act<true, false, 4>) : (drop ? k_bio_act<false, true, 4> : k_bio_act<false, false, 4>))
              : (bwd ? (drop ? k_bio_act<true, true, 1> : k_bio_act<true, false, 1>) : (drop ? k_bio_act<false, true, 1> : k_bio_act<false, false, 1>));
  PGNN_CUDA(pgnn_launch(k, dim3(grid_items(M * 32, 256)), dim3(256), 0, st, x, ldx, z, ldz, M, C, relu, d, y, ldy));
  PGNN_LAUNCH_CHECK();
  return PGNN_OK;
}

int bio_act_bwd(const float*& gz, int64_t& ldgz, const float* gy, int64_t ldgy, const float* z, int64_t M, int64_t D, bool last,
                const PgnnDropout& d, float* buf, cudaStream_t st) {
  if (last && d.p == 0.f && ldgy % 4 == 0 && aligned16(gy)) {
    gz = gy;
    ldgz = ldgy;
    return PGNN_OK;
  }
  gz = buf;
  ldgz = D;
  return bio_act(true, gy, ldgy, z, D, M, D, !last, d, buf, D, st);
}

int bio_pack_tables(int type, const void* const* params, int64_t L, int64_t C, float* T, cudaStream_t st) {
  const int PL = bio_layer_params(type), ew = bio_enc_w(type);
  for (int64_t l0 = 0; l0 < L; l0 += kMaxPack) {
    const int count = (int)(L - l0 < kMaxPack ? L - l0 : kMaxPack);
    PackArgs a{};
    for (int i = 0; i < count; ++i) {
      const void* const* p = params + PB_LAYER0 + (l0 + i) * PL;
      a.w[i] = (const float*)p[ew];
      a.b[i] = (const float*)p[ew + 1];
      PGNN_CHECK_ARG(a.w[i] && a.b[i]);
    }
    PGNN_CUDA(pgnn_launch(k_bio_pack_tables, dim3(grid_items(kBioQ * C * count, 256)), dim3(256), 0, st, a, count, (int)C,
                          T + l0 * kBioQ * C));
    PGNN_LAUNCH_CHECK();
  }
  return PGNN_OK;
}

struct BioGinWs : Front {
  float* T;
  double* bn_acc;
  float *mean, *invstd;
  float *aggr, *z1, *y1, *z2;
  float *gz2, *gy1, *gz1, *ga;
  float *gh, *gT;
  float* wpart;
  int64_t wpart_floats;
  void* scratch;
  int64_t scratch_bytes, total;
};

BioGinWs carve_bio_gin(void* base, int64_t N, int64_t E, int64_t L, int64_t D) {
  Carve c(base, false);
  BioGinWs w;
  const int64_t D2 = 2 * D;
  carve_front(c, w, kGin, N, E, D, kBioQ, 0);
  w.T = c.take<float>(L * kBioQ * D);
  w.bn_acc = c.take<double>(L * 2 * D2);
  w.mean = c.take<float>(L * D2);
  w.invstd = c.take<float>(L * D2);
  w.aggr = c.take<float>(L * N * D2);
  w.z1 = c.take<float>(L * N * D2);
  w.y1 = c.take<float>(L * N * D2);
  w.z2 = c.take<float>(L * N * D);
  w.gz2 = c.take<float>(2 * N * D);
  w.gy1 = c.take<float>(N * D2);
  w.gz1 = c.take<float>(2 * N * D2);
  w.ga = c.take<float>(N * D2);
  w.gh = c.take<float>(N * D);
  w.gT = c.take<float>(L * kBioQ * D);
  const int64_t a = pgnn_tc_wgrad_workspace_floats(N, D2, D2), b = pgnn_tc_wgrad_workspace_floats(N, D, D2);
  w.wpart_floats = a > b ? a : b;
  w.wpart = c.take<float>(w.wpart_floats);
  int64_t sb = pgnn_graph_prep_workspace_bytes(N, E);
  const int64_t bb = pgnn_bn_workspace_bytes(N > 0 ? N : 1, D2);
  if (bb > sb) sb = bb;
  w.scratch_bytes = sb;
  w.scratch = c.take<char>(sb);
  w.total = c.off;
  return w;
}

struct BioConvWs : Front {
  float *T, *xl, *z, *hout;
  float *nrm, *alpha, *pq;
  float *gz, *ga, *gxl, *gh;
  float* gT;
  float* wpart;
  int64_t wpart_floats;
  void* scratch;
  int64_t scratch_bytes, total;
};

BioConvWs carve_bio_conv(void* base, int type, int64_t N, int64_t E, int64_t L, int64_t D) {
  Carve c(base, true);
  BioConvWs w;
  const int64_t C = bio_width(type, D);
  carve_front(c, w, type, N, E, D, kBioQ, 0);
  w.T = c.take<float>(L * kBioQ * C);
  w.xl = c.take<float>(L * N * C);
  w.z = c.take<float>(L * N * D);
  w.hout = c.take<float>(L * N * D);
  w.nrm = c.take<float>(type == PGNN_CONV_SAGE ? L * N : 0);
  w.alpha = c.take<float>(type == PGNN_CONV_GAT ? L * (E + N) * kHeads : 0);
  w.pq = c.take<float>(type == PGNN_CONV_GAT ? L * N * kHeads * 2 : 0);
  w.gz = c.take<float>(N * D);
  w.ga = c.take<float>(N * D);
  w.gxl = c.take<float>(2 * N * C);
  w.gh = c.take<float>(N * D);
  w.gT = c.take<float>(L * kBioQ * C);
  w.wpart_floats = pgnn_tc_wgrad_workspace_floats(N, C, D);
  w.wpart = c.take<float>(w.wpart_floats);
  int64_t sb = pgnn_graph_prep_workspace_bytes(N, E);
  if (type == PGNN_CONV_GAT) {
    const int64_t gb = pgnn_gat_bwd_workspace_bytes(N, E, kHeads, D);
    if (gb > sb) sb = gb;
  }
  w.scratch_bytes = sb;
  w.scratch = c.take<char>(sb);
  w.total = c.off;
  return w;
}

int64_t bio_workspace_bytes(int type, int64_t N, int64_t E, int64_t L, int64_t D) {
  return type == kGin ? carve_bio_gin(nullptr, N, E, L, D).total : carve_bio_conv(nullptr, type, N, E, L, D).total;
}

int bio_prologue(int type, const Front& f, float* T, const void* const* params, const float* x, const int64_t* edge_index,
                 const float* edge_attr, int64_t N, int64_t E, int64_t L, int64_t D, void* scratch, int64_t scratch_bytes, cudaStream_t st) {
  TRY(pgnn_graph_prep(edge_index, E, N, f.rowptr_t, f.nbr_t, f.eid_t, f.rowptr_s, f.nbr_s, f.eid_s, scratch, scratch_bytes, st));
  if (type == PGNN_CONV_GCN) TRY(pgnn_gcn_dinv(f.rowptr_t, N, f.dinv, st));
  if (type != PGNN_CONV_GAT) TRY(pgnn_bio_edge_summary(edge_attr, f.rowptr_t, f.nbr_t, f.eid_t, N, agg_mode(type), f.dinv, f.S, st));
  TRY(pgnn_bio_embed_fwd(x, (const float*)params[PB_EMB], N, D, f.h0, D, st));
  return bio_pack_tables(type, params, L, bio_width(type, D), T, st);
}

int side_wgrad(const SideCtx* sc, cudaStream_t st, int k, int par, int precision, const float* gy, int64_t ldgy, const float* x,
               int64_t ldx, int64_t M, int64_t Nout, int64_t K, float* gw, float* gb, float* wpart, int64_t wpart_floats) {
  cudaStream_t wst = sc ? sc->side : st;
  if (sc) {
    PGNN_CUDA(cudaEventRecord(sc->ready[k][par], st));
    PGNN_CUDA(cudaStreamWaitEvent(wst, sc->ready[k][par], 0));
  }
  int rc = PGNN_EUNSUPPORTED;
  if (precision == 1) rc = pgnn_tc_linear_bwd_w_ws(gy, ldgy, x, ldx, M, Nout, K, gw, gb, wpart, wpart_floats, wst);
  if (rc == PGNN_EUNSUPPORTED) {
    if (sc) TRY(join_side(sc, st));
    return pgnn_linear_bwd_w(gy, ldgy, x, ldx, M, Nout, K, gw, gb, precision, st);
  }
  if (rc == PGNN_OK && sc) PGNN_CUDA(cudaEventRecord(sc->done[k][par], wst));
  return rc;
}

int bio_backward_tail(int type, const SideCtx* sc, const float* gT, const float* gh, const float* x, int64_t N, int64_t L, int64_t D,
                      float* grads, const int64_t* off, cudaStream_t st) {
  if (sc) TRY(join_side(sc, st));
  TRY(pgnn_bio_embed_bwd(x, gh, D, N, D, grads + off[PB_EMB], st));
  const int64_t C = bio_width(type, D);
  const int64_t stride = off[PB_LAYER0 + bio_layer_params(type)] - off[PB_LAYER0];
  PGNN_CUDA(pgnn_launch(k_bio_unpack_table_grads, dim3(grid_items(L * kBioQ * C, 256)), dim3(256), 0, st, gT, L, (int)C,
                        grads + off[PB_LAYER0 + bio_enc_w(type)], stride));
  PGNN_LAUNCH_CHECK();
  return PGNN_OK;
}

int bio_gin_forward(const void* const* params, void* const* bn_running_mean, void* const* bn_running_var, void* const* bn_num_batches_tracked,
                    int64_t N, int64_t L, int64_t D, int training, float momentum, float eps, const Drops& drops, int precision,
                    float* node_rep, int64_t ld_out, const BioGinWs& w, cudaStream_t st) {
  const int64_t D2 = 2 * D;
  for (int64_t l = 0; l < L; ++l) {
    const void* const* p = params + PB_LAYER0 + l * BG_COUNT;
    float* aggr = w.aggr + l * N * D2;
    float* z1 = w.z1 + l * N * D2;
    float* y1 = w.y1 + l * N * D2;
    float* z2 = w.z2 + l * N * D;
    const bool last = l == L - 1;
    const PgnnDropout drop_in = drops.at(l > 0 ? l - 1 : 0), drop_out = drops.at(l);
    const float* h = l == 0 ? w.h0 : w.z2 + (l - 1) * N * D;
    TRY(pgnn_internal_aggregate_fwd(h, D, nullptr, nullptr, l > 0, N, D, w.rowptr_t, w.nbr_t, PGNN_AGG_SUM, nullptr, w.S, kBioQ,
                                    w.T + l * kBioQ * D, nullptr, kBioQ, D, aggr, D2, st, nullptr, l > 0 ? &drop_in : nullptr));
    const float* gamma = (const float*)p[BG_GAMMA];
    const float* beta = (const float*)p[BG_BETA];
    float* rm = (float*)bn_running_mean[l];
    float* rv = (float*)bn_running_var[l];
    int64_t* nbt = bn_num_batches_tracked ? (int64_t*)bn_num_batches_tracked[l] : nullptr;
    double* acc = w.bn_acc + l * 2 * D2;
    bool stats_fused = false;
    if (training && precision == 1) {
      PGNN_CUDA(cudaMemsetAsync(acc, 0, sizeof(double) * 2 * D2, st));
      PgnnGemmHooks hk;
      hk.stats = acc;
      const int rc = pgnn_tc_linear_fwd(aggr, D2, (const float*)p[BG_W1], (const float*)p[BG_B1], N, D2, D2, 0, z1, D2, st, &hk);
      if (rc == PGNN_OK) stats_fused = true;
      else if (rc != PGNN_EUNSUPPORTED) return rc;
    }
    if (!stats_fused) TRY(pgnn_linear_fwd(aggr, D2, (const float*)p[BG_W1], (const float*)p[BG_B1], N, D2, D2, 0, z1, D2, precision, st));
    if (stats_fused) {
      PgnnBnFold fold{};
      fold.acc = acc; fold.gamma = gamma; fold.beta = beta;
      fold.running_mean = rm; fold.running_var = rv; fold.nbt = nbt;
      fold.save_mean = w.mean + l * D2; fold.save_invstd = w.invstd + l * D2;
      fold.momentum = momentum; fold.eps = eps; fold.set_rows((int)N);
      TRY(pgnn_internal_bn_apply_fold(z1, D2, N, D2, fold, 1, y1, D2, st, nullptr));
    } else if (training) {
      TRY(pgnn_internal_bn_fwd_train(z1, D2, N, D2, gamma, beta, rm, rv, nbt, momentum, eps, 1, y1, D2, w.mean + l * D2, w.invstd + l * D2,
                                     nullptr, nullptr, w.scratch, w.scratch_bytes, st, nullptr));
    } else {
      TRY(pgnn_bn_fwd_eval(z1, D2, N, D2, gamma, beta, rm, rv, eps, 1, y1, D2, st));
    }
    const bool direct = last && drop_out.p == 0.f;
    TRY(pgnn_linear_fwd(y1, D2, (const float*)p[BG_W2], (const float*)p[BG_B2], N, D, D2, 0, direct ? node_rep : z2, direct ? ld_out : D,
                        precision, st));
    if (last && !direct) TRY(bio_act(false, z2, D, nullptr, 0, N, D, 0, drop_out, node_rep, ld_out, st));
  }
  return PGNN_OK;
}

int bio_gin_backward(const void* const* params, const float* g_node_rep, int64_t ldg, const float* x, int64_t N, int64_t L, int64_t D,
                     const Drops& drops, int precision, float* grads, const int64_t* off, const BioGinWs& w, cudaStream_t st) {
  const int64_t D2 = 2 * D;
  SideCtx* sc = precision == 1 ? side_ctx(st) : nullptr;
  PGNN_CUDA(cudaMemsetAsync(w.gT, 0, sizeof(float) * L * kBioQ * D, st));
  const float* gy = g_node_rep;
  int64_t ldgy = ldg;
  for (int64_t l = L - 1; l >= 0; --l) {
    const void* const* p = params + PB_LAYER0 + l * BG_COUNT;
    const int64_t* o = off + PB_LAYER0 + l * BG_COUNT;
    const bool last = l == L - 1;
    const int par = (int)(l & 1);
    const float* aggr = w.aggr + l * N * D2;
    const float* z1 = w.z1 + l * N * D2;
    const float* y1 = w.y1 + l * N * D2;
    float* gz2 = w.gz2 + (sc ? par * N * D : 0);
    float* gz1 = w.gz1 + (sc ? par * N * D2 : 0);
    if (sc) PGNN_CUDA(cudaStreamWaitEvent(st, sc->done[0][par], 0));
    const float* gz;
    int64_t ldgz;
    TRY(bio_act_bwd(gz, ldgz, gy, ldgy, w.z2 + l * N * D, N, D, last, drops.at(l), gz2, st));
    TRY(side_wgrad(sc, st, 0, par, precision, gz, ldgz, y1, D2, N, D, D2, grads + o[BG_W2], grads + o[BG_B2], w.wpart, w.wpart_floats));
    TRY(pgnn_linear_bwd_x(gz, ldgz, (const float*)p[BG_W2], N, D, D2, nullptr, 0, w.gy1, D2, precision, st));
    if (sc) PGNN_CUDA(cudaStreamWaitEvent(st, sc->done[1][par], 0));
    TRY(pgnn_internal_bn_bwd(w.gy1, D2, z1, D2, N, D2, (const float*)p[BG_GAMMA], (const float*)p[BG_BETA], w.mean + l * D2,
                             w.invstd + l * D2, 1, gz1, D2, grads + o[BG_GAMMA], grads + o[BG_BETA], grads + o[BG_B1], w.scratch,
                             w.scratch_bytes, st, nullptr));
    TRY(side_wgrad(sc, st, 1, par, precision, gz1, D2, aggr, D2, N, D2, D2, grads + o[BG_W1], nullptr, w.wpart, w.wpart_floats));
    TRY(pgnn_linear_bwd_x(gz1, D2, (const float*)p[BG_W1], N, D2, D2, nullptr, 0, w.ga, D2, precision, st));
    TRY(pgnn_internal_edge_table_bwd2(w.S, kBioQ, w.ga, D2, D, N, (int)D, w.gT + l * kBioQ * D, D, nullptr, kBioQ, st));
    TRY(pgnn_aggregate_bwd(w.ga, D2, N, D, w.rowptr_s, w.nbr_s, PGNN_AGG_SUM, nullptr, w.rowptr_t, w.gh, D, st));
    gy = w.gh;
    ldgy = D;
  }
  return bio_backward_tail(kGin, sc, w.gT, w.gh, x, N, L, D, grads, off, st);
}

int bio_conv_forward(int type, const void* const* params, const float* edge_attr, int64_t N, int64_t E, int64_t L, int64_t D,
                     const Drops& drops, int precision, float* node_rep, int64_t ld_out, const BioConvWs& w, cudaStream_t st) {
  const bool gat = type == PGNN_CONV_GAT;
  const int64_t C = bio_width(type, D);
  const int PL = bio_layer_params(type);
  const float* h = w.h0;
  for (int64_t l = 0; l < L; ++l) {
    const void* const* p = params + PB_LAYER0 + l * PL;
    const bool last = l == L - 1;
    const PgnnDropout drop = drops.at(l);
    float* xl = w.xl + l * N * C;
    float* z = w.z + l * N * D;
    const float* T = w.T + l * kBioQ * C;
    const bool direct = last && drop.p == 0.f && type != PGNN_CONV_SAGE && ld_out % 4 == 0 && aligned16(node_rep);
    float* out = direct ? node_rep : z;
    const int64_t ldo = direct ? ld_out : D;
    TRY(pgnn_linear_fwd(h, D, (const float*)p[gat ? BA_W : BC_W], (const float*)p[gat ? BA_B : BC_B], N, C, D, 0, xl, C, precision, st));
    if (gat) {
      TRY(pgnn_gat_fwd(xl, N, kHeads, D, (const float*)p[BA_ATT], T, 1, edge_attr, w.rowptr_t, w.nbr_t, w.eid_t, E, (const float*)p[BA_BIAS],
                       kSlope, w.alpha + l * (E + N) * kHeads, w.pq + l * N * kHeads * 2, out, ldo, st));
    } else if (type == PGNN_CONV_GCN) {
      TRY(pgnn_internal_aggregate_fwd(xl, D, nullptr, nullptr, 0, N, D, w.rowptr_t, w.nbr_t, PGNN_AGG_GCN, w.dinv, w.S, kBioQ, T, nullptr,
                                      kBioQ, 0, out, ldo, st, nullptr, nullptr));
    } else {
      TRY(pgnn_internal_aggregate_fwd(xl, D, nullptr, nullptr, 0, N, D, w.rowptr_t, w.nbr_t, PGNN_AGG_MEAN, nullptr, w.S, kBioQ, T, nullptr,
                                      kBioQ, 0, w.gz, D, st, nullptr, nullptr));
      TRY(pgnn_l2norm_fwd(w.gz, D, N, D, z, D, w.nrm + l * N, st));
    }
    float* hout = w.hout + l * N * D;
    if (!last) TRY(bio_act(false, z, D, nullptr, 0, N, D, 1, drop, hout, D, st));
    else if (!direct) TRY(bio_act(false, z, D, nullptr, 0, N, D, 0, drop, node_rep, ld_out, st));
    h = hout;
  }
  return PGNN_OK;
}

int bio_conv_backward(int type, const void* const* params, const float* g_node_rep, int64_t ldg, const float* x, const float* edge_attr,
                      int64_t N, int64_t E, int64_t L, int64_t D, const Drops& drops, int precision, float* grads, const int64_t* off,
                      const BioConvWs& w, cudaStream_t st) {
  const bool gat = type == PGNN_CONV_GAT;
  const int64_t C = bio_width(type, D);
  const int PL = bio_layer_params(type);
  SideCtx* sc = precision == 1 ? side_ctx(st) : nullptr;
  if (!gat) PGNN_CUDA(cudaMemsetAsync(w.gT, 0, sizeof(float) * L * kBioQ * C, st));
  const float* gy = g_node_rep;
  int64_t ldgy = ldg;
  for (int64_t l = L - 1; l >= 0; --l) {
    const void* const* p = params + PB_LAYER0 + l * PL;
    const int64_t* o = off + PB_LAYER0 + l * PL;
    const bool last = l == L - 1;
    const int par = (int)(l & 1);
    const float* xl = w.xl + l * N * C;
    const float* z = w.z + l * N * D;
    const float* hin = l == 0 ? w.h0 : w.hout + (l - 1) * N * D;
    float* gxl = w.gxl + (sc ? par * N * C : 0);
    float* gT = w.gT + l * kBioQ * C;
    const float* gz;
    int64_t ldgz;
    TRY(bio_act_bwd(gz, ldgz, gy, ldgy, z, N, D, last, drops.at(l), w.gz, st));
    if (sc) PGNN_CUDA(cudaStreamWaitEvent(st, sc->done[0][par], 0));
    if (gat) {
      TRY(pgnn_gat_bwd(gz, ldgz, xl, N, kHeads, D, (const float*)p[BA_ATT], w.T + l * kBioQ * C, 1, edge_attr, w.rowptr_t, w.nbr_t, w.eid_t,
                       w.rowptr_s, w.nbr_s, w.eid_s, E, kSlope, w.alpha + l * (E + N) * kHeads, w.pq + l * N * kHeads * 2, gxl,
                       grads + o[BA_ATT], gT, grads + o[BA_BIAS], w.scratch, w.scratch_bytes, st));
    } else {
      const float* ga = gz;
      int64_t ldga = ldgz;
      if (type == PGNN_CONV_SAGE) {
        TRY(pgnn_l2norm_bwd(gz, ldgz, z, D, w.nrm + l * N, N, D, w.ga, D, st));
        ga = w.ga;
        ldga = D;
      }
      TRY(pgnn_internal_edge_table_bwd2(w.S, kBioQ, ga, ldga, 0, N, (int)D, gT, D, nullptr, kBioQ, st));
      TRY(pgnn_aggregate_bwd(ga, ldga, N, D, w.rowptr_s, w.nbr_s, agg_mode(type), w.dinv, w.rowptr_t, gxl, D, st));
    }
    TRY(side_wgrad(sc, st, 0, par, precision, gxl, C, hin, D, N, C, D, grads + o[gat ? BA_W : BC_W], grads + o[gat ? BA_B : BC_B], w.wpart,
                   w.wpart_floats));
    TRY(pgnn_linear_bwd_x(gxl, C, (const float*)p[gat ? BA_W : BC_W], N, C, D, nullptr, 0, w.gh, D, precision, st));
    gy = w.gh;
    ldgy = D;
  }
  return bio_backward_tail(type, sc, w.gT, w.gh, x, N, L, D, grads, off, st);
}

}

extern "C" {

int64_t pgnn_chem_gin_num_params(int64_t L) { return L < 1 ? PGNN_EINVAL : grad_layout(kGin, L, 0, nullptr); }

int pgnn_chem_gin_grad_offsets(int64_t L, int64_t D, int64_t* offsets ) {
  PGNN_CHECK_ARG(L >= 1 && D > 0 && offsets);
  grad_layout(kGin, L, D, offsets);
  return PGNN_OK;
}

int64_t pgnn_chem_gin_workspace_bytes(int64_t N, int64_t E, int64_t L, int64_t D) {
  if (N < 0 || E < 0 || L < 1 || D <= 0) return PGNN_EINVAL;
  return carve_gin(nullptr, N, E, L, D).total;
}

int pgnn_chem_gin_forward(const void* const* params, void* const* bn_running_mean, void* const* bn_running_var,
                          void* const* bn_num_batches_tracked, const int64_t* x, const int64_t* edge_index,
                          const int64_t* edge_attr, int64_t N, int64_t E, int64_t L, int64_t D, int training, float momentum, float eps,
                          int precision, float* node_rep, int64_t ld_out, void* workspace, int64_t workspace_bytes, void* stream) {
  return pgnn_chem_encoder_forward(kGin, params, bn_running_mean, bn_running_var, bn_num_batches_tracked, x, edge_index, edge_attr, N, E, L, D,
                                   training, momentum, eps, 0.f, 0, precision, node_rep, ld_out, workspace, workspace_bytes, stream);
}

int pgnn_chem_gin_backward(const void* const* params, const float* g_node_rep, int64_t ldg, const int64_t* x, int64_t N, int64_t E,
                           int64_t L, int64_t D, int precision, float* grads, void* workspace, int64_t workspace_bytes,
                           void* stream) {
  return pgnn_chem_encoder_backward(kGin, params, g_node_rep, ldg, x, nullptr, N, E, L, D, 0.f, 0, precision, grads, workspace,
                                    workspace_bytes, stream);
}

int pgnn_chem_gin_debug_layout(int64_t N, int64_t E, int64_t L, int64_t D, int64_t* out4) {
  PGNN_CHECK_ARG(N >= 0 && E >= 0 && L >= 1 && D > 0 && out4);
  char* base = reinterpret_cast<char*>(0x1000);
  GinWs w = carve_gin(base, N, E, L, D);
  out4[0] = reinterpret_cast<char*>(w.z1) - base;
  out4[1] = reinterpret_cast<char*>(w.z2) - base;
  out4[2] = reinterpret_cast<char*>(w.mean) - base;
  out4[3] = reinterpret_cast<char*>(w.invstd) - base;
  return PGNN_OK;
}

int64_t pgnn_chem_gin_debug_aggr_offset(int64_t N, int64_t E, int64_t L, int64_t D) {
  if (N < 0 || E < 0 || L < 1 || D <= 0) return PGNN_EINVAL;
  char* base = reinterpret_cast<char*>(0x1000);
  GinWs w = carve_gin(base, N, E, L, D);
  return reinterpret_cast<char*>(w.aggr) - base;
}

int64_t pgnn_chem_conv_num_params(int conv_type, int64_t L) {
  if (!valid_conv(conv_type) || L < 1) return PGNN_EINVAL;
  return grad_layout(conv_type, L, 0, nullptr);
}

int pgnn_chem_conv_grad_offsets(int conv_type, int64_t L, int64_t D, int64_t* offsets) {
  PGNN_CHECK_ARG(valid_conv(conv_type) && L >= 1 && D > 0 && offsets);
  grad_layout(conv_type, L, D, offsets);
  return PGNN_OK;
}

int64_t pgnn_chem_conv_workspace_bytes(int conv_type, int64_t N, int64_t E, int64_t L, int64_t D) {
  if (!valid_conv(conv_type) || N < 0 || E < 0 || L < 1 || D <= 0) return PGNN_EINVAL;
  return carve_conv(nullptr, conv_type, N, E, L, D).total;
}

int pgnn_chem_conv_forward(int conv_type, const void* const* params, void* const* bn_running_mean, void* const* bn_running_var,
                           void* const* bn_num_batches_tracked, const int64_t* x, const int64_t* edge_index, const int64_t* edge_attr,
                           int64_t N, int64_t E, int64_t L, int64_t D, int training, float momentum, float eps, int precision,
                           float* node_rep, int64_t ld_out, void* workspace, int64_t workspace_bytes, void* stream) {
  PGNN_CHECK_ARG(valid_conv(conv_type));
  return pgnn_chem_encoder_forward(conv_type, params, bn_running_mean, bn_running_var, bn_num_batches_tracked, x, edge_index, edge_attr, N, E, L,
                                   D, training, momentum, eps, 0.f, 0, precision, node_rep, ld_out, workspace, workspace_bytes, stream);
}

int pgnn_chem_conv_backward(int conv_type, const void* const* params, const float* g_node_rep, int64_t ldg, const int64_t* x,
                            const int64_t* edge_attr, int64_t N, int64_t E, int64_t L, int64_t D, int precision, float* grads,
                            void* workspace, int64_t workspace_bytes, void* stream) {
  PGNN_CHECK_ARG(valid_conv(conv_type));
  return pgnn_chem_encoder_backward(conv_type, params, g_node_rep, ldg, x, edge_attr, N, E, L, D, 0.f, 0, precision, grads, workspace,
                                    workspace_bytes, stream);
}

int pgnn_chem_encoder_forward(int gnn_type, const void* const* params, void* const* bn_running_mean, void* const* bn_running_var,
                              void* const* bn_num_batches_tracked, const int64_t* x, const int64_t* edge_index, const int64_t* edge_attr,
                              int64_t N, int64_t E, int64_t L, int64_t D, int training, float momentum, float eps, float drop_p,
                              int64_t drop_seed, int precision, float* node_rep, int64_t ld_out, void* workspace, int64_t workspace_bytes,
                              void* stream) {
  PGNN_CHECK_ARG((gnn_type == kGin || valid_conv(gnn_type)) && drop_p >= 0.f && drop_p <= 1.f);
  Drops drops;
  if (training) drops = Drops{drop_p, drop_seed};
  if (gnn_type == kGin)
    return gin_forward(params, bn_running_mean, bn_running_var, bn_num_batches_tracked, x, edge_index, edge_attr, N, E, L, D, training, momentum,
                       eps, drops, precision, node_rep, ld_out, workspace, workspace_bytes, stream);
  return conv_forward(gnn_type, params, bn_running_mean, bn_running_var, bn_num_batches_tracked, x, edge_index, edge_attr, N, E, L, D, training,
                      momentum, eps, drops, precision, node_rep, ld_out, workspace, workspace_bytes, stream);
}

int pgnn_chem_encoder_backward(int gnn_type, const void* const* params, const float* g_node_rep, int64_t ldg, const int64_t* x,
                               const int64_t* edge_attr, int64_t N, int64_t E, int64_t L, int64_t D, float drop_p, int64_t drop_seed,
                               int precision, float* grads, void* workspace, int64_t workspace_bytes, void* stream) {
  PGNN_CHECK_ARG((gnn_type == kGin || valid_conv(gnn_type)) && drop_p >= 0.f && drop_p <= 1.f);
  const Drops drops{drop_p, drop_seed};
  if (gnn_type == kGin)
    return gin_backward(params, g_node_rep, ldg, x, N, E, L, D, drops, precision, grads, workspace, workspace_bytes, stream);
  return conv_backward(gnn_type, params, g_node_rep, ldg, x, edge_attr, N, E, L, D, drops, precision, grads, workspace, workspace_bytes,
                       stream);
}

int64_t pgnn_bio_encoder_num_params(int gnn_type, int64_t L) {
  if (!valid_type(gnn_type) || L < 1) return PGNN_EINVAL;
  return bio_grad_layout(gnn_type, L, 0, nullptr);
}

int pgnn_bio_encoder_grad_offsets(int gnn_type, int64_t L, int64_t D, int64_t* offsets) {
  PGNN_CHECK_ARG(valid_type(gnn_type) && L >= 1 && D > 0 && offsets);
  bio_grad_layout(gnn_type, L, D, offsets);
  return PGNN_OK;
}

int64_t pgnn_bio_encoder_workspace_bytes(int gnn_type, int64_t N, int64_t E, int64_t L, int64_t D) {
  if (!valid_type(gnn_type) || N < 0 || E < 0 || L < 1 || D <= 0) return PGNN_EINVAL;
  return bio_workspace_bytes(gnn_type, N, E, L, D);
}

int pgnn_bio_encoder_forward(int gnn_type, const void* const* params, void* const* bn_running_mean, void* const* bn_running_var,
                             void* const* bn_num_batches_tracked, const float* x, const int64_t* edge_index, const float* edge_attr,
                             int64_t N, int64_t E, int64_t L, int64_t D, int training, float momentum, float eps, float drop_p,
                             int64_t drop_seed, int precision, float* node_rep, int64_t ld_out, void* workspace, int64_t workspace_bytes,
                             void* stream) {
  PGNN_CHECK_ARG(valid_type(gnn_type) && drop_p >= 0.f && drop_p <= 1.f);
  PGNN_CHECK_ARG(N >= 0 && E >= 0 && L >= 1 && D > 0 && D % 4 == 0 && params && workspace);
  PGNN_CHECK_ARG(gnn_type != kGin || (bn_running_mean && bn_running_var));
  PGNN_CHECK_ARG(N == 0 || (x && node_rep && ld_out >= D));
  PGNN_CHECK_ARG(E == 0 || (edge_index && edge_attr));
  if (workspace_bytes < bio_workspace_bytes(gnn_type, N, E, L, D)) return PGNN_EWORKSPACE;
  if (N == 0) return PGNN_OK;
  Drops drops;
  if (training) drops = Drops{drop_p, drop_seed};
  cudaStream_t st = as_stream(stream);
  if (gnn_type == kGin) {
    const BioGinWs w = carve_bio_gin(workspace, N, E, L, D);
    TRY(bio_prologue(kGin, w, w.T, params, x, edge_index, edge_attr, N, E, L, D, w.scratch, w.scratch_bytes, st));
    return bio_gin_forward(params, bn_running_mean, bn_running_var, bn_num_batches_tracked, N, L, D, training, momentum, eps, drops,
                           precision, node_rep, ld_out, w, st);
  }
  const BioConvWs w = carve_bio_conv(workspace, gnn_type, N, E, L, D);
  TRY(bio_prologue(gnn_type, w, w.T, params, x, edge_index, edge_attr, N, E, L, D, w.scratch, w.scratch_bytes, st));
  return bio_conv_forward(gnn_type, params, edge_attr, N, E, L, D, drops, precision, node_rep, ld_out, w, st);
}

int pgnn_bio_encoder_backward(int gnn_type, const void* const* params, const float* g_node_rep, int64_t ldg, const float* x,
                              const float* edge_attr, int64_t N, int64_t E, int64_t L, int64_t D, float drop_p, int64_t drop_seed,
                              int precision, float* grads, void* workspace, int64_t workspace_bytes, void* stream) {
  PGNN_CHECK_ARG(valid_type(gnn_type) && drop_p >= 0.f && drop_p <= 1.f);
  PGNN_CHECK_ARG(N >= 0 && E >= 0 && L >= 1 && D > 0 && D % 4 == 0 && params && grads && workspace);
  if (workspace_bytes < bio_workspace_bytes(gnn_type, N, E, L, D)) return PGNN_EWORKSPACE;
  const int64_t count = bio_grad_layout(gnn_type, L, D, nullptr);
  std::vector<int64_t> offsets(count + 1);
  bio_grad_layout(gnn_type, L, D, offsets.data());
  cudaStream_t st = as_stream(stream);
  if (N == 0) {
    PGNN_CUDA(cudaMemsetAsync(grads, 0, sizeof(float) * offsets[count], st));
    return PGNN_OK;
  }
  PGNN_CHECK_ARG(g_node_rep && x && ldg >= D && (E == 0 || gnn_type != PGNN_CONV_GAT || edge_attr));
  const Drops drops{drop_p, drop_seed};
  if (gnn_type == kGin)
    return bio_gin_backward(params, g_node_rep, ldg, x, N, L, D, drops, precision, grads, offsets.data(),
                            carve_bio_gin(workspace, N, E, L, D), st);
  return bio_conv_backward(gnn_type, params, g_node_rep, ldg, x, edge_attr, N, E, L, D, drops, precision, grads, offsets.data(),
                           carve_bio_conv(workspace, gnn_type, N, E, L, D), st);
}

}
```

Before: 141,900.

## Pre-split weights into padded tf32 hi/lo images and stream them with cp.async

```diff
diff --git a/include/pgnn_b200.h b/include/pgnn_b200.h
--- a/include/pgnn_b200.h
+++ b/include/pgnn_b200.h
@@ -182,6 +182,12 @@
 PGNN_API int pgnn_debug_tc_wgrad_plan(int64_t M, int64_t N, int64_t K, int64_t* out4);
 PGNN_API int pgnn_debug_transpose_batch(int count, const float* const* in, float* const* out, const int32_t* rows,
                                         const int32_t* cols, void* stream);
+PGNN_API int pgnn_debug_pack_weight_images(int count, const float* const* w, const int64_t* ld, const int32_t* rows,
+                                           const int32_t* cols, const int32_t* transposed, float* const* img, void* stream);
+PGNN_API int pgnn_debug_tc_gemm_img(int bn, const float* A, int64_t lda, const float* B, int64_t ldb, float* img, float* C,
+                                    int64_t ldc, int64_t M, int64_t N, int64_t K, const float* bias, int relu, const float* mask,
+                                    int64_t ldm, float* colsum, double* stats, const float* S, int Q, float* gT, float* gT2,
+                                    int q_split, int64_t ldt, void* stream);
 PGNN_API int pgnn_debug_bn_apply_fold(const float* x, int64_t ldx, int64_t M, int64_t C, const double* sums, const float* gamma,
                                       const float* beta, float* running_mean, float* running_var, int64_t* num_batches_tracked,
                                       float momentum, float eps, float* save_mean, float* save_invstd, int relu, float* y, int64_t ldy,
diff --git a/pretrain-gnns_b200/csrc/dense_tc.cu b/pretrain-gnns_b200/csrc/dense_tc.cu
--- a/pretrain-gnns_b200/csrc/dense_tc.cu
+++ b/pretrain-gnns_b200/csrc/dense_tc.cu
@@ -71,6 +71,10 @@
 
 __device__ __forceinline__ int kperm(int k) { return (k & 16) | ((k & 3) << 2) | ((k >> 2) & 3); }
 
+constexpr int kImgRows = 128;
+__host__ __device__ constexpr int64_t img_rows(int64_t rows) { return (rows + kImgRows - 1) / kImgRows * kImgRows; }
+__host__ __device__ constexpr int64_t img_ld(int64_t k) { return (k + BK - 1) / BK * BK; }
+
 __device__ __forceinline__ int araw_off(int m, int k) { return k * BM + (m ^ ((((k >> 2) & 3) << 3) ^ ((k & 1) << 4))); }
 
 __device__ __forceinline__ int akc_off(int m, int k) { return m * BK + ((((k >> 2) ^ ((m & 1) << 2))) << 2) + (k & 3); }
@@ -176,19 +180,37 @@
     const float* src = n > 0 ? (KC ? A + (int64_t)gr * lda + k0 + kk : A + (int64_t)(k0 + kk) * lda + gr) : A;
     cp_async16(dst + (KC ? akc_off(rr, kk) : araw_off(rr, kk)), src, 4 * n);
   }
-  cp_async_commit();
-}
+}
+
+template <int BN>
+__device__ __forceinline__ void b_img_copy(uint8_t* hi, uint8_t* lo, const float* __restrict__ img, int64_t ld, int64_t plane, int n0,
+                                           int k0) {
+#pragma unroll
+  for (int i = 0; i < Loader<true, BN>::NV; ++i) {
+    const int f = threadIdx.x + i * NTHREADS, rr = f >> 3, kk = (f & 7) * 4;
+    const float* src = img + (int64_t)(n0 + rr) * ld + k0 + kk;
+    const int o = sw128_off(rr, kk);
+    cp_async16(reinterpret_cast<float*>(hi + o), src, 16);
+    cp_async16(reinterpret_cast<float*>(lo + o), src + plane, 16);
+  }
+}
+
+template <int N>
+__device__ __forceinline__ void cp_async_wait() { asm volatile("cp.async.wait_group %0;" ::"n"(N) : "memory"); }
 
 constexpr int NSTAGE = 3;
 
-template <int BN>
+template <int BN, bool B_IMG = false>
 struct TileCfg {
   static constexpr int B_BYTES = BN * BK * 4;
   static constexpr int STAGE = 2 * B_BYTES;
   static constexpr int A_RAW = BM * BK * 4;
+  static constexpr int B_STAGES = B_IMG ? 4 : NSTAGE;
+  static constexpr int A_DIST = B_IMG && BN == 128 ? 2 : 1;
+  static constexpr int A_BUFS = A_DIST + 1;
   static constexpr int SLD = BN + 4;
   static constexpr int EPI = BM * SLD * 4 + BM * kMaxHookQ * 4;
-  static constexpr int RING = NSTAGE * STAGE + 2 * A_RAW;
+  static constexpr int RING = B_STAGES * STAGE + A_BUFS * A_RAW;
   static constexpr int SMEM = (RING > EPI ? RING : EPI) + 1024;
   static constexpr int FRAG_SETS = BN == 128 ? 4 : 2;
   static constexpr int MIN_BLOCKS = BN <= 64 ? 2 : 1;
@@ -298,20 +320,22 @@
   }
 }
 
-template <bool A_KC, bool B_KC, int BN>
-__global__ void __launch_bounds__(NTHREADS, TileCfg<BN>::MIN_BLOCKS)
+template <bool A_KC, bool B_KC, int BN, bool B_IMG>
+__global__ void __launch_bounds__(NTHREADS, TileCfg<BN, B_IMG>::MIN_BLOCKS)
 k_gemm_3xtf32(const float* __restrict__ A, int64_t lda, const float* __restrict__ B, int64_t ldb, float* __restrict__ C, int64_t ldc,
               int M, int N, int K, int k_per_split, TcEpilogue ep) {
   static_assert(BN == 64 || BN == 128, "one wgmma.m64nBNk8 per product; two accumulators of BN / 2 registers each");
-  using Cfg = TileCfg<BN>;
+  static_assert(!B_IMG || (A_KC && B_KC), "the image path serves the forward and dgrad GEMMs: K-major A and B");
+  using Cfg = TileCfg<BN, B_IMG>;
   constexpr int NF = Cfg::FRAG_SETS;
+  constexpr int NB = Cfg::B_STAGES, NA = Cfg::A_BUFS;
   static_assert((BK / 8) % NF == 0, "k-step j uses fragment set j % NF in every block");
   extern __shared__ uint8_t smem_raw[];
   __shared__ __align__(16) float s_bias[BN];
   uint8_t* smem = smem_raw + ((1024 - (smem_u32(smem_raw) & 1023)) & 1023);
   auto b_hi = [&](int s) { return smem + s * Cfg::STAGE; };
   auto b_lo = [&](int s) { return b_hi(s) + Cfg::B_BYTES; };
-  float* a_raw = reinterpret_cast<float*>(smem + NSTAGE * Cfg::STAGE);
+  float* a_raw = reinterpret_cast<float*>(smem + NB * Cfg::STAGE);
 
   const int warp = threadIdx.x >> 5, lane = threadIdx.x & 31, wg = threadIdx.x >> 7;
   const int t = lane & 3;
@@ -326,7 +350,8 @@
   for (int i = threadIdx.x; i < BN; i += NTHREADS) s_bias[i] = (s_bias_on && n0 + i < N) ? ep.bias[n0 + i] : 0.f;
 
   Loader<B_KC, BN> lb;
-  lb.init(B, ldb, n0, N, kbeg);
+  if constexpr (!B_IMG) lb.init(B, ldb, n0, N, kbeg);
+  const int64_t plane = B_IMG ? img_rows(N) * ldb : 0;
 
   float acc[BN / 2], accx[BN / 2];
 #pragma unroll
@@ -335,21 +360,47 @@
 
   if (nkb > 0) {
     a_copy<A_KC>(a_raw, A, lda, m0, M, kbeg, kend - kbeg);
-    lb.load(0, kend - kbeg);
-    lb.store(b_hi(0), b_lo(0));
-    asm volatile("fence.proxy.async.shared::cta;" ::: "memory");
-    cp_async_wait_all();
-  }
-  int s = 0;
+    if constexpr (B_IMG) {
+      b_img_copy<BN>(b_hi(0), b_lo(0), B, ldb, plane, n0, kbeg);
+      cp_async_commit();
+      if (nkb > 1) {
+        if (Cfg::A_DIST == 2) a_copy<A_KC>(a_raw + BM * BK, A, lda, m0, M, kbeg + BK, kend - kbeg - BK);
+        b_img_copy<BN>(b_hi(1), b_lo(1), B, ldb, plane, n0, kbeg + BK);
+      }
+      cp_async_commit();
+      cp_async_wait<1>();
+      asm volatile("fence.proxy.async.shared::cta;" ::: "memory");
+    } else {
+      cp_async_commit();
+      lb.load(0, kend - kbeg);
+      lb.store(b_hi(0), b_lo(0));
+      asm volatile("fence.proxy.async.shared::cta;" ::: "memory");
+      cp_async_wait_all();
+    }
+  }
+  int s = 0, sa = 0;
 #pragma unroll 1
   for (int kb = 0; kb < nkb; ++kb) {
     __syncthreads();
     const bool more = kb + 1 < nkb;
-    if (more) {
+    if constexpr (B_IMG) {
+      if (Cfg::A_DIST == 1) {
+        const int k1 = kbeg + (kb + 1) * BK;
+        if (more) a_copy<A_KC>(a_raw + (sa ^ 1) * (BM * BK), A, lda, m0, M, k1, kend - k1);
+        cp_async_commit();
+      }
+      if (kb + 2 < nkb) {
+        const int k2 = kbeg + (kb + 2) * BK, s2 = s + 2 < NB ? s + 2 : s + 2 - NB;
+        if (Cfg::A_DIST == 2) a_copy<A_KC>(a_raw + (sa == 0 ? NA - 1 : sa - 1) * (BM * BK), A, lda, m0, M, k2, kend - k2);
+        b_img_copy<BN>(b_hi(s2), b_lo(s2), B, ldb, plane, n0, k2);
+      }
+      cp_async_commit();
+    } else if (more) {
       a_copy<A_KC>(a_raw + ((kb + 1) & 1) * (BM * BK), A, lda, m0, M, kbeg + (kb + 1) * BK, kend - kbeg - (kb + 1) * BK);
+      cp_async_commit();
       lb.load(kb + 1, kend - kbeg - (kb + 1) * BK);
     }
-    const float* ar = a_raw + (kb & 1) * (BM * BK);
+    const float* ar = a_raw + (B_IMG ? sa : kb & 1) * (BM * BK);
     float4 av[2];
     const uint64_t dh = gmma_desc_sw128(smem_u32(b_hi(s))), dl = gmma_desc_sw128(smem_u32(b_lo(s)));
 #pragma unroll
@@ -380,13 +431,20 @@
       wgmma_tf32_rs<BN>(acc, fh[f], dh + 2 * j);
       wgmma_commit();
     }
-    s = s + 1 == NSTAGE ? 0 : s + 1;
+    s = s + 1 == NB ? 0 : s + 1;
+    if constexpr (B_IMG) sa = sa + 1 == NA ? 0 : sa + 1;
     if (more) {
-      lb.store(b_hi(s), b_lo(s));
-      asm volatile("fence.proxy.async.shared::cta;" ::: "memory");
-      cp_async_wait_all();
-    }
-  }
+      if constexpr (B_IMG) {
+        cp_async_wait<1>();
+        asm volatile("fence.proxy.async.shared::cta;" ::: "memory");
+      } else {
+        lb.store(b_hi(s), b_lo(s));
+        asm volatile("fence.proxy.async.shared::cta;" ::: "memory");
+        cp_async_wait_all();
+      }
+    }
+  }
+  if constexpr (B_IMG) cp_async_wait_all();
   wgmma_wait<0>();
   fence_acc(acc);
   fence_acc(accx);
@@ -427,20 +485,20 @@
   }
 }
 
-template <bool A_KC, bool B_KC, int BN>
+template <bool A_KC, bool B_KC, int BN, bool B_IMG = false>
 int launch(const float* A, int64_t lda, const float* B, int64_t ldb, float* C, int64_t ldc, int M, int N, int K, int splits,
            int k_per_split, const TcEpilogue& ep, cudaStream_t st) {
-  constexpr int smem = TileCfg<BN>::SMEM;
+  constexpr int smem = TileCfg<BN, B_IMG>::SMEM;
   static std::atomic<uint64_t> configured{0};
   int dev = 0;
   PGNN_CUDA(cudaGetDevice(&dev));
   const uint64_t bit = dev < 64 ? (uint64_t)1 << dev : 0;
   if (!(configured.load(std::memory_order_relaxed) & bit)) {
-    PGNN_CUDA(cudaFuncSetAttribute(k_gemm_3xtf32<A_KC, B_KC, BN>, cudaFuncAttributeMaxDynamicSharedMemorySize, smem));
+    PGNN_CUDA(cudaFuncSetAttribute(k_gemm_3xtf32<A_KC, B_KC, BN, B_IMG>, cudaFuncAttributeMaxDynamicSharedMemorySize, smem));
     configured.fetch_or(bit, std::memory_order_relaxed);
   }
   dim3 grid((unsigned)ceil_div(N, BN), (unsigned)ceil_div(M, BM), (unsigned)splits);
-  PGNN_CUDA(pgnn_launch(k_gemm_3xtf32<A_KC, B_KC, BN>, dim3(grid), dim3(NTHREADS), smem, st, A, lda, B, ldb, C, ldc, M, N, K, k_per_split, ep));
+  PGNN_CUDA(pgnn_launch(k_gemm_3xtf32<A_KC, B_KC, BN, B_IMG>, dim3(grid), dim3(NTHREADS), smem, st, A, lda, B, ldb, C, ldc, M, N, K, k_per_split, ep));
   PGNN_LAUNCH_CHECK();
   return PGNN_OK;
 }
@@ -459,22 +517,103 @@
   return launch<A_KC, B_KC, 128>(A, lda, B, ldb, C, ldc, M, N, K, splits, k_per_split, ep, st);
 }
 
-}
-
-extern "C" int pgnn_debug_tc_gemm(int a_kc, int b_kc, int bn, const float* A, int64_t lda, const float* B, int64_t ldb, float* C,
-                                  int64_t ldc, int64_t M, int64_t N, int64_t K, const float* bias, int relu, const float* mask,
-                                  int64_t ldm, float* colsum, double* stats, const float* S, int Q, float* gT, float* gT2,
-                                  int q_split, int64_t ldt, void* stream) {
-  PGNN_CHECK_ARG(bn == 64 || bn == 128);
-  PGNN_CHECK_ARG(M > 0 && N > 0 && K > 0 && M < (1ll << 31) && N < (1ll << 31) && K < (1ll << 31));
-  PGNN_CHECK_ARG(A && B && C && ldc >= N && lda >= (a_kc ? K : M) && ldb >= (b_kc ? K : N));
+int dispatch_img(int bn, const float* A, int64_t lda, const float* img, float* C, int64_t ldc, int M, int N, int K, const TcEpilogue& ep,
+                 cudaStream_t st) {
+  if (ep.hooks.S && (ep.hooks.Q < 1 || ep.hooks.Q > kMaxHookQ)) return PGNN_EINVAL;
+  if (bn == 64) return launch<true, true, 64, true>(A, lda, img, img_ld(K), C, ldc, M, N, K, 1, K, ep, st);
+  return launch<true, true, 128, true>(A, lda, img, img_ld(K), C, ldc, M, N, K, 1, K, ep, st);
+}
+
+struct PackJob { const float* w; float* img; int64_t ld; int rows, cols, trans; };
+constexpr int kMaxPackJobs = 32;
+struct PackBatch { PackJob job[kMaxPackJobs]; };
+__global__ void __launch_bounds__(256) k_pack_img_batch(PackBatch b) {
+  pdl_prologue();
+  __shared__ float tile[32][33];
+  const PackJob j = b.job[blockIdx.z];
+  const int R = j.trans ? j.cols : j.rows, Kr = j.trans ? j.rows : j.cols;
+  const int64_t ld = img_ld(Kr), nr = img_rows(R);
+  const int k0 = blockIdx.x * 32, r0 = blockIdx.y * 32;
+  if (k0 >= ld || r0 >= nr) return;
+  const int tx = threadIdx.x & 31, ty = threadIdx.x >> 5;
+  for (int i = ty; i < 32; i += 8) {
+    if (j.trans) {
+      const int r = r0 + tx, k = k0 + i;
+      tile[tx][i] = r < R && k < Kr ? j.w[(int64_t)k * j.ld + r] : 0.f;
+    } else {
+      const int r = r0 + i, k = k0 + tx;
+      tile[i][tx] = r < R && k < Kr ? j.w[(int64_t)r * j.ld + k] : 0.f;
+    }
+  }
+  __syncthreads();
+  const int rr = threadIdx.x >> 3, c = (threadIdx.x & 7) * 4;
+  float h[4], l[4];
+#pragma unroll
+  for (int q = 0; q < 4; ++q) split_tf32(tile[rr][kperm(c + q)], h[q], l[q]);
+  float* dst = j.img + (int64_t)(r0 + rr) * ld + k0 + c;
+  *reinterpret_cast<float4*>(dst) = make_float4(h[0], h[1], h[2], h[3]);
+  *reinterpret_cast<float4*>(dst + nr * ld) = make_float4(l[0], l[1], l[2], l[3]);
+}
+
+}
+
+int64_t pgnn_tc_image_floats(int64_t rows, int64_t k) { return 2 * img_rows(rows) * img_ld(k); }
+
+int pgnn_internal_pack_images(int count, const float* const* w, const int64_t* ld, const int* rows, const int* cols, const int* trans,
+                              float* const* img, cudaStream_t st) {
+  if (count <= 0) return PGNN_OK;
+  if (count > kMaxPackJobs) return PGNN_EUNSUPPORTED;
+  PackBatch b;
+  int64_t mr = 0, mk = 0;
+  for (int i = 0; i < count; ++i) {
+    if (!aligned16(img[i])) return PGNN_EUNSUPPORTED;
+    b.job[i] = PackJob{w[i], img[i], ld[i], rows[i], cols[i], trans[i] ? 1 : 0};
+    const int64_t R = img_rows(trans[i] ? cols[i] : rows[i]), K = img_ld(trans[i] ? rows[i] : cols[i]);
+    mr = R > mr ? R : mr;
+    mk = K > mk ? K : mk;
+  }
+  dim3 grid((unsigned)(mk / 32), (unsigned)(mr / 32), (unsigned)count);
+  PGNN_CUDA(pgnn_launch(k_pack_img_batch, dim3(grid), dim3(256), 0, st, b));
+  PGNN_LAUNCH_CHECK();
+  return PGNN_OK;
+}
+
+int pgnn_tc_linear_fwd_img(const float* x, int64_t ldx, const float* img, int64_t img_r, int64_t img_k, const float* bias, int64_t M,
+                           int64_t N, int64_t K, int relu, float* y, int64_t ldy, cudaStream_t st, const PgnnGemmHooks* hooks) {
+  if (img_r != img_rows(N) || img_k != img_ld(K)) return PGNN_EINVAL;
+  if (ldx % 4 || !aligned16(x) || !aligned16(img) || !aligned16(y) || M < 1) return PGNN_EUNSUPPORTED;
+  TcEpilogue ep{bias, relu, nullptr, 0, 0, hooks ? *hooks : PgnnGemmHooks{}};
+  return dispatch_img(pick_bn((int)M, (int)N, 1), x, ldx, img, y, ldy, (int)M, (int)N, (int)K, ep, st);
+}
+
+int pgnn_tc_linear_bwd_x_img(const float* gy, int64_t ldgy, const float* img, int64_t img_r, int64_t img_k, int64_t M, int64_t N,
+                             int64_t K, const float* relu_src, int64_t ldr, float* gx, int64_t ldgx, cudaStream_t st,
+                             const PgnnGemmHooks* hooks) {
+  if (img_r != img_rows(K) || img_k != img_ld(N)) return PGNN_EINVAL;
+  if (ldgy % 4 || !aligned16(gy) || !aligned16(img) || !aligned16(gx) || M < 1) return PGNN_EUNSUPPORTED;
+  TcEpilogue ep{nullptr, 0, relu_src, ldr, 0, hooks ? *hooks : PgnnGemmHooks{}};
+  return dispatch_img(pick_bn((int)M, (int)K, 1), gy, ldgy, img, gx, ldgx, (int)M, (int)K, (int)N, ep, st);
+}
+
+extern "C" int pgnn_debug_pack_weight_images(int count, const float* const* w, const int64_t* ld, const int32_t* rows,
+                                             const int32_t* cols, const int32_t* transposed, float* const* img, void* stream) {
+  PGNN_CHECK_ARG(count >= 0);
+  if (count == 0) return PGNN_OK;
+  PGNN_CHECK_ARG(w && ld && rows && cols && transposed && img);
+  if (count > kMaxPackJobs) return PGNN_EUNSUPPORTED;
+  for (int i = 0; i < count; ++i) PGNN_CHECK_ARG(w[i] && img[i] && rows[i] > 0 && cols[i] > 0 && ld[i] >= cols[i]);
+  return pgnn_internal_pack_images(count, w, ld, rows, cols, transposed, img, as_stream(stream));
+}
+
+namespace {
+int debug_epilogue(int64_t N, const float* bias, int relu, const float* mask, int64_t ldm, float* colsum, double* stats, const float* S,
+                   int Q, float* gT, float* gT2, int q_split, int64_t ldt, TcEpilogue& ep) {
   PGNN_CHECK_ARG(!mask || ldm >= N);
   if (S) {
     PGNN_CHECK_ARG(Q >= 1 && Q <= kMaxHookQ && q_split >= 0 && q_split <= Q && ldt >= N);
     PGNN_CHECK_ARG((q_split == 0 || gT) && (q_split == Q || gT2));
   }
-  if (lda % 4 || ldb % 4 || !aligned16(A) || !aligned16(B)) return PGNN_EUNSUPPORTED;
-  TcEpilogue ep{bias, relu, mask, ldm, 0, PgnnGemmHooks{}};
+  ep = TcEpilogue{bias, relu, mask, ldm, 0, PgnnGemmHooks{}};
   ep.hooks.colsum = colsum;
   ep.hooks.stats = stats;
   ep.hooks.S = S;
@@ -483,6 +622,39 @@
   ep.hooks.gT2 = gT2;
   ep.hooks.q_split = q_split;
   ep.hooks.ldt = ldt;
+  return PGNN_OK;
+}
+}
+
+extern "C" int pgnn_debug_tc_gemm_img(int bn, const float* A, int64_t lda, const float* B, int64_t ldb, float* img, float* C, int64_t ldc,
+                                      int64_t M, int64_t N, int64_t K, const float* bias, int relu, const float* mask, int64_t ldm,
+                                      float* colsum, double* stats, const float* S, int Q, float* gT, float* gT2, int q_split,
+                                      int64_t ldt, void* stream) {
+  PGNN_CHECK_ARG(bn == 64 || bn == 128);
+  PGNN_CHECK_ARG(M > 0 && N > 0 && K > 0 && M < (1ll << 31) && N < (1ll << 31) && K < (1ll << 31));
+  PGNN_CHECK_ARG(A && B && img && C && ldc >= N && lda >= K && ldb >= K);
+  TcEpilogue ep;
+  const int rc = debug_epilogue(N, bias, relu, mask, ldm, colsum, stats, S, Q, gT, gT2, q_split, ldt, ep);
+  if (rc != PGNN_OK) return rc;
+  if (lda % 4 || ldb % 4 || !aligned16(A) || !aligned16(B) || !aligned16(img)) return PGNN_EUNSUPPORTED;
+  cudaStream_t st = as_stream(stream);
+  const int r = (int)N, c = (int)K, zero = 0;
+  const int prc = pgnn_internal_pack_images(1, &B, &ldb, &r, &c, &zero, &img, st);
+  if (prc != PGNN_OK) return prc;
+  return dispatch_img(bn, A, lda, img, C, ldc, (int)M, (int)N, (int)K, ep, st);
+}
+
+extern "C" int pgnn_debug_tc_gemm(int a_kc, int b_kc, int bn, const float* A, int64_t lda, const float* B, int64_t ldb, float* C,
+                                  int64_t ldc, int64_t M, int64_t N, int64_t K, const float* bias, int relu, const float* mask,
+                                  int64_t ldm, float* colsum, double* stats, const float* S, int Q, float* gT, float* gT2,
+                                  int q_split, int64_t ldt, void* stream) {
+  PGNN_CHECK_ARG(bn == 64 || bn == 128);
+  PGNN_CHECK_ARG(M > 0 && N > 0 && K > 0 && M < (1ll << 31) && N < (1ll << 31) && K < (1ll << 31));
+  PGNN_CHECK_ARG(A && B && C && ldc >= N && lda >= (a_kc ? K : M) && ldb >= (b_kc ? K : N));
+  TcEpilogue ep;
+  const int rc = debug_epilogue(N, bias, relu, mask, ldm, colsum, stats, S, Q, gT, gT2, q_split, ldt, ep);
+  if (rc != PGNN_OK) return rc;
+  if (lda % 4 || ldb % 4 || !aligned16(A) || !aligned16(B)) return PGNN_EUNSUPPORTED;
   cudaStream_t st = as_stream(stream);
   const int m = (int)M, n = (int)N, k = (int)K;
   if (a_kc && b_kc) return dispatch<true, true>(bn, A, lda, B, ldb, C, ldc, m, n, k, 1, k, ep, st);
@@ -503,13 +675,6 @@
   if (K % 4 || ldgy % 4 || !aligned16(gy) || !aligned16(w) || !aligned16(gx) || M < 1) return PGNN_EUNSUPPORTED;
   TcEpilogue ep{nullptr, 0, relu_src, ldr, 0, hooks ? *hooks : PgnnGemmHooks{}};
   return dispatch<true, false>(pick_bn((int)M, (int)K, 1), gy, ldgy, w, K, gx, ldgx, (int)M, (int)K, (int)N, 1, (int)N, ep, st);
-}
-
-int pgnn_tc_linear_bwd_x_wt(const float* gy, int64_t ldgy, const float* wT, int64_t M, int64_t N, int64_t K, const float* relu_src,
-                            int64_t ldr, float* gx, int64_t ldgx, cudaStream_t st, const PgnnGemmHooks* hooks) {
-  if (N % 4 || ldgy % 4 || !aligned16(gy) || !aligned16(wT) || !aligned16(gx) || M < 1) return PGNN_EUNSUPPORTED;
-  TcEpilogue ep{nullptr, 0, relu_src, ldr, 0, hooks ? *hooks : PgnnGemmHooks{}};
-  return dispatch<true, true>(pick_bn((int)M, (int)K, 1), gy, ldgy, wT, N, gx, ldgx, (int)M, (int)K, (int)N, 1, (int)N, ep, st);
 }
 
 namespace {
diff --git a/pretrain-gnns_b200/csrc/encoder.cu b/pretrain-gnns_b200/csrc/encoder.cu
--- a/pretrain-gnns_b200/csrc/encoder.cu
+++ b/pretrain-gnns_b200/csrc/encoder.cu
@@ -22,10 +22,14 @@
 int pgnn_tc_linear_bwd_w_ws(const float* gy, int64_t ldgy, const float* x, int64_t ldx, int64_t M, int64_t N, int64_t K, float* gw,
                             float* gb, float* partials, int64_t partial_floats, cudaStream_t st);
 int64_t pgnn_tc_wgrad_workspace_floats(int64_t M, int64_t N, int64_t K);
-int pgnn_tc_linear_bwd_x_wt(const float* gy, int64_t ldgy, const float* wT, int64_t M, int64_t N, int64_t K, const float* relu_src,
-                            int64_t ldr, float* gx, int64_t ldgx, cudaStream_t st, const PgnnGemmHooks* hooks);
-int pgnn_internal_transpose_batch(int count, const float* const* in, float* const* out, const int* rows, const int* cols,
-                                  cudaStream_t st);
+int64_t pgnn_tc_image_floats(int64_t rows, int64_t k);
+int pgnn_internal_pack_images(int count, const float* const* w, const int64_t* ld, const int* rows, const int* cols, const int* trans,
+                              float* const* img, cudaStream_t st);
+int pgnn_tc_linear_fwd_img(const float* x, int64_t ldx, const float* img, int64_t img_r, int64_t img_k, const float* bias, int64_t M,
+                           int64_t N, int64_t K, int relu, float* y, int64_t ldy, cudaStream_t st, const PgnnGemmHooks* hooks);
+int pgnn_tc_linear_bwd_x_img(const float* gy, int64_t ldgy, const float* img, int64_t img_r, int64_t img_k, int64_t M, int64_t N,
+                             int64_t K, const float* relu_src, int64_t ldr, float* gx, int64_t ldgx, cudaStream_t st,
+                             const PgnnGemmHooks* hooks);
 int pgnn_internal_bn_apply_fold(const float* x, int64_t ldx, int64_t M, int64_t C, const PgnnBnFold& fold, int relu, float* y,
                                 int64_t ldy, cudaStream_t st, const PgnnDropout* drop);
 int pgnn_internal_bn_fwd_train(const float* x, int64_t ldx, int64_t M, int64_t C, const float* gamma, const float* beta,
@@ -144,7 +148,7 @@
   double* bn_acc;
   float *aggr, *z1, *z2;
   float *gh, *gz2, *gz1, *gaggr;
-  float* wT;
+  float* wimg;
   float* wpart;
   int64_t wpart_floats;
   void* scratch;
@@ -167,7 +171,7 @@
   w.gz2 = c.take<float>(2 * N * D);
   w.gz1 = c.take<float>(2 * N * 2 * D);
   w.gaggr = c.take<float>(N * D);
-  w.wT = c.take<float>(L * 4 * D * D);
+  w.wimg = c.take<float>(L * (pgnn_tc_image_floats(2 * D, D) + pgnn_tc_image_floats(D, 2 * D)));
   w.wpart_floats = split_k_floats(N, 2 * D, D);
   w.wpart = c.take<float>(w.wpart_floats);
   int64_t sb = pgnn_graph_prep_workspace_bytes(N, E);
@@ -177,6 +181,49 @@
   w.scratch = c.take<char>(sb);
   w.total = c.off;
   return w;
+}
+
+struct GinImages {
+  bool on = false;
+  const float* base = nullptr;
+  int64_t D = 0;
+  static int64_t rows_pad(int64_t rows) { return align_up(rows, 128); }
+  static int64_t k_pad(int64_t k) { return align_up(k, 32); }
+  const float* wide(int64_t l) const { return base + l * (pgnn_tc_image_floats(2 * D, D) + pgnn_tc_image_floats(D, 2 * D)); }
+  const float* narrow(int64_t l) const { return wide(l) + pgnn_tc_image_floats(2 * D, D); }
+};
+
+int pack_gin_images(const GinWs& w, const void* const* params, int64_t L, int64_t D, bool transposed, cudaStream_t st, GinImages& im) {
+  im = GinImages{};
+  const char* e = getenv("PGNN_WEIGHT_IMAGES");
+  if (2 * L > 32 || (e && e[0] == '0')) return PGNN_OK;
+  im.base = w.wimg;
+  im.D = D;
+  const float* src[32];
+  float* dst[32];
+  int64_t ld[32];
+  int rows[32], cols[32], tr[32];
+  for (int64_t l = 0; l < L; ++l) {
+    const void* const* p = params + P_LAYER0 + l * L_COUNT;
+    const float* w1 = (const float*)p[L_W1];
+    const float* w2 = (const float*)p[L_W2];
+    const int i = (int)(2 * l);
+    src[i] = transposed ? w2 : w1;
+    src[i + 1] = transposed ? w1 : w2;
+    dst[i] = const_cast<float*>(im.wide(l));
+    dst[i + 1] = const_cast<float*>(im.narrow(l));
+    rows[i] = (int)(transposed ? D : 2 * D);
+    cols[i] = (int)(transposed ? 2 * D : D);
+    rows[i + 1] = (int)(transposed ? 2 * D : D);
+    cols[i + 1] = (int)(transposed ? D : 2 * D);
+    ld[i] = cols[i];
+    ld[i + 1] = cols[i + 1];
+    tr[i] = tr[i + 1] = transposed ? 1 : 0;
+  }
+  const int rc = pgnn_internal_pack_images((int)(2 * L), src, ld, rows, cols, tr, dst, st);
+  if (rc == PGNN_OK) im.on = true;
+  else if (rc != PGNN_EUNSUPPORTED) return rc;
+  return PGNN_OK;
 }
 
 struct ConvWs : Front {
@@ -295,6 +342,11 @@
   if (N == 0) return PGNN_OK;
   GinWs w = carve_gin(workspace, N, E, L, D);
   TRY(forward_prologue(kGin, w, params, x, edge_index, edge_attr, N, E, D, training, precision, w.scratch, w.scratch_bytes, stream));
+  cudaStream_t st = as_stream(stream);
+  GinImages im;
+  if (precision == 1) TRY(pack_gin_images(w, params, L, D, false, st, im));
+  const int64_t wide_r = GinImages::rows_pad(2 * D), wide_k = GinImages::k_pad(D);
+  const int64_t narrow_r = GinImages::rows_pad(D), narrow_k = GinImages::k_pad(2 * D);
   const float* h = w.h0;
   const float *in_scale = nullptr, *in_shift = nullptr;
   PgnnBnFold fold;
@@ -310,7 +362,12 @@
     TRY(pgnn_internal_aggregate_fwd(h, D, in_scale, in_shift, in_scale != nullptr || have_fold, N, D, w.rowptr_t, w.nbr_t, PGNN_AGG_SUM,
                                     nullptr, w.S, 9, (const float*)p[L_ET1], (const float*)p[L_ET2], 6, 0, aggr, D, as_stream(stream),
                                     have_fold ? &fold : nullptr, l > 0 ? &drop_in : nullptr));
-    TRY(pgnn_linear_fwd(aggr, D, (const float*)p[L_W1], (const float*)p[L_B1], N, 2 * D, D, 1, z1, 2 * D, precision, stream));
+    int rc1 = im.on ? pgnn_tc_linear_fwd_img(aggr, D, im.wide(l), wide_r, wide_k, (const float*)p[L_B1], N, 2 * D, D, 1, z1, 2 * D, st,
+                                             nullptr)
+                    : PGNN_EUNSUPPORTED;
+    if (rc1 == PGNN_EUNSUPPORTED)
+      rc1 = pgnn_linear_fwd(aggr, D, (const float*)p[L_W1], (const float*)p[L_B1], N, 2 * D, D, 1, z1, 2 * D, precision, stream);
+    if (rc1 != PGNN_OK) return rc1;
     have_fold = false;
     bool stats_fused = false;
     double* acc = bn_acc + l * 2 * D;
@@ -318,12 +375,22 @@
       PGNN_CUDA(cudaMemsetAsync(acc, 0, sizeof(double) * 2 * D, as_stream(stream)));
       PgnnGemmHooks hk;
       hk.stats = acc;
-      const int rc = pgnn_tc_linear_fwd(z1, 2 * D, (const float*)p[L_W2], (const float*)p[L_B2], N, D, 2 * D, 0, z2, D, as_stream(stream), &hk);
+      int rc = im.on ? pgnn_tc_linear_fwd_img(z1, 2 * D, im.narrow(l), narrow_r, narrow_k, (const float*)p[L_B2], N, D, 2 * D, 0, z2, D,
+                                              st, &hk)
+                     : PGNN_EUNSUPPORTED;
+      if (rc == PGNN_EUNSUPPORTED)
+        rc = pgnn_tc_linear_fwd(z1, 2 * D, (const float*)p[L_W2], (const float*)p[L_B2], N, D, 2 * D, 0, z2, D, st, &hk);
       if (rc == PGNN_OK) stats_fused = true;
       else if (rc != PGNN_EUNSUPPORTED) return rc;
     }
-    if (!stats_fused)
-      TRY(pgnn_linear_fwd(z1, 2 * D, (const float*)p[L_W2], (const float*)p[L_B2], N, D, 2 * D, 0, z2, D, precision, stream));
+    if (!stats_fused) {
+      int rc = im.on && !training ? pgnn_tc_linear_fwd_img(z1, 2 * D, im.narrow(l), narrow_r, narrow_k, (const float*)p[L_B2], N, D,
+                                                           2 * D, 0, z2, D, st, nullptr)
+                                  : PGNN_EUNSUPPORTED;
+      if (rc == PGNN_EUNSUPPORTED)
+        rc = pgnn_linear_fwd(z1, 2 * D, (const float*)p[L_W2], (const float*)p[L_B2], N, D, 2 * D, 0, z2, D, precision, stream);
+      if (rc != PGNN_OK) return rc;
+    }
     if (training && stats_fused) {
       fold = PgnnBnFold{};
       fold.acc = acc; fold.gamma = (const float*)p[L_GAMMA]; fold.beta = (const float*)p[L_BETA];
@@ -372,20 +439,10 @@
   }
   PGNN_CHECK_ARG(g_node_rep && x);
   GinWs w = carve_gin(workspace, N, E, L, D);
-  bool have_wT = false;
-  if (precision == 1 && 2 * L <= 32) {
-    const float* in[32];
-    float* out[32];
-    int rows[32], cols[32];
-    for (int64_t l = 0; l < L; ++l) {
-      const void* const* p = params + P_LAYER0 + l * L_COUNT;
-      in[2 * l] = (const float*)p[L_W1];     out[2 * l] = w.wT + (2 * l) * 2 * D * D;     rows[2 * l] = (int)(2 * D); cols[2 * l] = (int)D;
-      in[2 * l + 1] = (const float*)p[L_W2]; out[2 * l + 1] = w.wT + (2 * l + 1) * 2 * D * D; rows[2 * l + 1] = (int)D; cols[2 * l + 1] = (int)(2 * D);
-    }
-    const int rc = pgnn_internal_transpose_batch((int)(2 * L), in, out, rows, cols, st);
-    if (rc == PGNN_OK) have_wT = true;
-    else if (rc != PGNN_EUNSUPPORTED) return rc;
-  }
+  GinImages im;
+  if (precision == 1) TRY(pack_gin_images(w, params, L, D, true, st, im));
+  const int64_t wide_r = GinImages::rows_pad(2 * D), wide_k = GinImages::k_pad(D);
+  const int64_t narrow_r = GinImages::rows_pad(D), narrow_k = GinImages::k_pad(2 * D);
   const float* gy = g_node_rep;
   int64_t ldgy = ldg;
   SideCtx* sc = precision == 1 ? side_ctx(st) : nullptr;
@@ -420,8 +477,8 @@
         PGNN_CUDA(cudaMemsetAsync(grads + o[L_B1], 0, sizeof(float) * 2 * D, st));
         PgnnGemmHooks h1;
         h1.colsum = grads + o[L_B1];
-        rc = have_wT ? pgnn_tc_linear_bwd_x_wt(gz2, D, w.wT + (2 * l + 1) * 2 * D * D, N, D, 2 * D, z1, 2 * D, gz1, 2 * D, st, &h1)
-                     : PGNN_EUNSUPPORTED;
+        rc = im.on ? pgnn_tc_linear_bwd_x_img(gz2, D, im.wide(l), wide_r, wide_k, N, D, 2 * D, z1, 2 * D, gz1, 2 * D, st, &h1)
+                   : PGNN_EUNSUPPORTED;
         if (rc == PGNN_EUNSUPPORTED)
           rc = pgnn_tc_linear_bwd_x(gz2, D, (const float*)p[L_W2], N, D, 2 * D, z1, 2 * D, gz1, 2 * D, st, &h1);
         if (rc != PGNN_OK) return rc;
@@ -435,8 +492,8 @@
         PGNN_CUDA(cudaMemsetAsync(grads + o[L_ET1], 0, sizeof(float) * 9 * D, st));
         PgnnGemmHooks h2;
         h2.S = w.S; h2.Q = 9; h2.gT = grads + o[L_ET1]; h2.gT2 = grads + o[L_ET2]; h2.q_split = 6; h2.ldt = D;
-        rc = have_wT ? pgnn_tc_linear_bwd_x_wt(gz1, 2 * D, w.wT + (2 * l) * 2 * D * D, N, 2 * D, D, nullptr, 0, w.gaggr, D, st, &h2)
-                     : PGNN_EUNSUPPORTED;
+        rc = im.on ? pgnn_tc_linear_bwd_x_img(gz1, 2 * D, im.narrow(l), narrow_r, narrow_k, N, 2 * D, D, nullptr, 0, w.gaggr, D, st, &h2)
+                   : PGNN_EUNSUPPORTED;
         if (rc == PGNN_EUNSUPPORTED)
           rc = pgnn_tc_linear_bwd_x(gz1, 2 * D, (const float*)p[L_W1], N, 2 * D, D, nullptr, 0, w.gaggr, D, st, &h2);
         if (rc != PGNN_OK) return rc;
```

Measured after the change: 154,100, median of 6. 8.6% higher.
